# Intelligent-Microsystems-Lab/SNNQuantPrune

Measured on AMD Instinct MI355X. Metric: samples/sec/node (DVS128 T=20, 4-bit/90%-pruned), higher is better.
Workload: dtype fp6*fp4->f32 (integer-exact); 1 GPU; C3 topology: 3x(qconv3x3+BN+LIF+pool2) + qdense(32768->110)+LIF + vote, DVS128 128x128x2, T=20, bits 4/4/4/4, 90% pruned; batch_per_gpu=1024, global_batch=1024, frames=20, parallelism=dp1 (batch-sharded, all-gather logits)

## Files before the change

include/snnqp.h:

```cpp
#ifndef SNNQP_H_
#define SNNQP_H_

#include <stdint.h>

#ifdef __cplusplus
extern "C" {
#endif

typedef void *snnqp_stream_t;

enum {
  SNNQP_OK = 0,
  SNNQP_EINVAL = -1,
  SNNQP_EUNSUPPORTED = -2,
  SNNQP_EHIP = -3
};

enum { SNNQP_F32 = 0, SNNQP_U8 = 1, SNNQP_BITS = 2, SNNQP_EV1 = 3, SNNQP_EV4 = 4 };
enum { SNNQP_W_F32 = 0, SNNQP_W_I8 = 1 };
enum {
  SNNQP_NEURON_NONE = 0,
  SNNQP_NEURON_MULTI_STEP_LIF = 1,
  SNNQP_NEURON_PARAMETRIC_LEAKY_IF = 2,
  SNNQP_NEURON_LIF = 3
};
enum {
  SNNQP_SURR_FAST_SIGMOID = 0,
  SNNQP_SURR_ATAN = 1,
  SNNQP_SURR_SLAYER = 2,
  SNNQP_SURR_SMOOTH_STEP = 3,
  SNNQP_SURR_PIECEWISE_LINEAR = 4
};
enum {
  SNNQP_Q_DUQ = 0,
  SNNQP_Q_UNIFORM_STATIC = 1,
  SNNQP_Q_PARAMETRIC_D = 2,
  SNNQP_Q_PARAMETRIC_D_XMAX = 3
};
enum { SNNQP_IMPL_AUTO = 0, SNNQP_IMPL_GENERIC = 1, SNNQP_IMPL_MFMA = 2 };

enum {
  SNNQP_FLAG_CODE_OVERFLOW = 1,
  SNNQP_FLAG_MASK_NOT_BINARY = 2,
  SNNQP_FLAG_NOT_INTEGER = 4,
  SNNQP_FLAG_GT_ONE = 8,
  SNNQP_FLAG_GT_127 = 16,
  SNNQP_FLAG_GT_15 = 32
};

typedef struct {
  int32_t wtype;
  const void *w;
  float L;
  float m;
  int32_t abs_sum_max;
  int32_t code_max;
  const int32_t *col_sum;
  const void *wt_fp6;
  uint32_t min_current_bits;
  int32_t ch_stack_max;
  const int32_t *ch_slots;
  int32_t wt_cin;
} snnqp_weight_t;

#define SNNQP_BN_MEAN_ZERO 1
#define SNNQP_BN_BIAS_ZERO 2
#define SNNQP_BN_MUL_UNIFORM 4
typedef struct {
  const float *mean;
  const float *mul;
  const float *bias;
  int32_t flags;
} snnqp_bn_t;

typedef struct {
  int32_t kind;
  float k;
  float v_threshold;
  float v_reset;
  const float *decay;
} snnqp_neuron_t;

typedef struct {
  int32_t H, W, Cin, Cout;
  int32_t KH, KW;
  int32_t stride_h, stride_w;
  int32_t pad_h_lo, pad_h_hi, pad_w_lo, pad_w_hi;
  int32_t in_dil_h, in_dil_w;
  int32_t k_dil_h, k_dil_w;
  int32_t groups;
} snnqp_conv_geom_t;

typedef struct {
  int32_t D, H, W, Cin, Cout;
  int32_t KD, KH, KW;
  int32_t stride[3];
  int32_t pad_lo[3], pad_hi[3];
  int32_t in_dil[3];
  int32_t k_dil[3];
  int32_t groups;
} snnqp_conv3d_geom_t;

#define SNNQP_VERSION 507
int snnqp_version(void);
const char *snnqp_last_error(void);
const char *snnqp_build_flags(void);

int snnqp_set_conv_k16(int enabled);

int snnqp_conv_out_shape(const snnqp_conv_geom_t *g, int32_t *OH, int32_t *OW);

int snnqp_quantize(int kind, const float *w, const float *mask, int64_t n,
                   int bits, float p0, float p1, float *fq_out,
                   int8_t *codes_out, int32_t *flags, snnqp_stream_t stream);
int snnqp_quantize_ex(int kind, const float *w, const float *mask, int64_t n,
                      int bits, int sign, float p0, float p1, float *fq_out,
                      int8_t *codes_out, int32_t *flags, snnqp_stream_t stream);

int snnqp_pack_codes_mfma(const int8_t *w, int64_t K, int32_t N, int32_t Npad,
                          int8_t *wt, snnqp_stream_t stream);

int snnqp_pack_codes_fp6(const int8_t *w, int64_t K, int32_t N, int32_t Npad, void *wt6,
                         snnqp_stream_t stream);

int snnqp_inspect_f32(const float *x, int64_t n, int32_t *flags,
                      snnqp_stream_t stream);
int snnqp_inspect_u8(const uint8_t *x, int64_t n, int32_t *flags,
                     snnqp_stream_t stream);
int snnqp_f32_to_u8(const float *x, uint8_t *y, int64_t n,
                    snnqp_stream_t stream);
int snnqp_narrow_f32(const float *x, uint8_t *y, int64_t n, int32_t *flags,
                     snnqp_stream_t stream);
int snnqp_pack_frames(const uint8_t *x, int64_t frames, int32_t H, int32_t W, int fmt,
                      void *y, int32_t *flags, snnqp_stream_t stream);
int snnqp_unpack_frames(const void *x, int fmt, int64_t frames, int32_t H, int32_t W,
                        uint8_t *y, snnqp_stream_t stream);
int snnqp_pack_frames_checked(const void *x, int in_type, int64_t frames, int32_t H, int32_t W,
                              uint32_t *y, int32_t *flags, snnqp_stream_t stream);
int snnqp_pack_bits(const void *x, int in_type, int64_t rows, int32_t C,
                    uint32_t *bits, snnqp_stream_t stream);
int snnqp_pack_bits_checked(const void *x, int in_type, int64_t rows, int32_t C,
                            uint32_t *bits, int32_t *flags, snnqp_stream_t stream);
int snnqp_unpack_bits(const uint32_t *bits, int64_t rows, int32_t C, float *y,
                      snnqp_stream_t stream);

int snnqp_conv_forward(const void *x, int in_type, int64_t NB,
                       const snnqp_conv_geom_t *g, const snnqp_weight_t *w,
                       float *y, int32_t *acc, snnqp_stream_t stream);
int snnqp_conv_forward_ex(const void *x, int in_type, int64_t NB,
                          const snnqp_conv_geom_t *g, const snnqp_weight_t *w,
                          const int8_t *wt, float *y, int32_t *acc, int impl,
                          snnqp_stream_t stream);
int snnqp_conv_forward_if(const int32_t *pred, const void *x, int in_type, int64_t NB,
                          const snnqp_conv_geom_t *g, const snnqp_weight_t *w, float *y,
                          snnqp_stream_t stream);

int snnqp_conv3d_out_shape(const snnqp_conv3d_geom_t *g, int32_t *OD, int32_t *OH, int32_t *OW);
int snnqp_conv3d_lif_forward(const int32_t *pred, const void *x, int in_type, int64_t x_stride_t,
                             int64_t x_stride_b, int32_t T, int32_t B,
                             const snnqp_conv3d_geom_t *g, const snnqp_weight_t *w,
                             const snnqp_bn_t *bn, const snnqp_neuron_t *nrn, const float *u0,
                             float *u_out, void *s_out, int s_type, snnqp_stream_t stream);

int64_t snnqp_conv_gated_packed_bytes(int32_t Cin, int32_t Cout);
int snnqp_pack_codes_gated(const int8_t *w, int32_t Cin, int32_t Cout, void *packed,
                           snnqp_stream_t stream);
int64_t snnqp_conv_gated_packed_bytes_ex(int32_t Cin, int32_t Cout, int32_t code_max);
int snnqp_pack_codes_gated_ex(const int8_t *w, int32_t Cin, int32_t Cout, int32_t code_max,
                              void *packed, snnqp_stream_t stream);
int snnqp_conv_gated_forward(const uint32_t *s, const float *gate, int64_t NB,
                             const snnqp_conv_geom_t *g, const snnqp_weight_t *w,
                             const void *packed, float *y, snnqp_stream_t stream);

int64_t snnqp_dense_gated_packed_bytes(int32_t C, int32_t N);
int snnqp_pack_codes_dense_gated(const int8_t *w, int32_t C, int32_t HW, int32_t N, void *packed,
                                 snnqp_stream_t stream);
int64_t snnqp_dense_gated_packed_bytes_ex(int32_t C, int32_t N, int32_t code_max);
int snnqp_pack_codes_dense_gated_ex(const int8_t *w, int32_t C, int32_t HW, int32_t N, int32_t code_max,
                                    void *packed, snnqp_stream_t stream);
int snnqp_dense_gated_forward(const uint32_t *s, const float *gate, int64_t NB, int32_t HW,
                              int32_t C, int32_t N, const snnqp_weight_t *w,
                              const void *packed, float *y, snnqp_stream_t stream);

int snnqp_conv_lif_forward(const void *x, int in_type, int64_t x_stride_t,
                           int64_t x_stride_b, int32_t T, int32_t B,
                           const snnqp_conv_geom_t *g, const snnqp_weight_t *w,
                           const int8_t *wt, const snnqp_bn_t *bn,
                           const snnqp_neuron_t *nrn, const float *u0,
                           float *u_out, void *s_out, int s_type, int pool,
                           int impl, int x_max, int32_t *x_seen, int32_t *x_flags,
                           snnqp_stream_t stream);
// ... 130 lines not shown
```

snnquantprune_amd/_lib.py:

```python

from __future__ import annotations

import ctypes
import os
from ctypes import (POINTER, Structure, c_char_p, c_float, c_int, c_int8,
                    c_int32, c_uint32, c_int64, c_void_p)

_HERE = os.path.dirname(os.path.abspath(__file__))
LIB_PATH = os.path.join(_HERE, "csrc", "libsnnqp.so")

ABI_VERSION = 507

F32, U8, BITS, EV1, EV4 = 0, 1, 2, 3, 4
W_F32, W_I8 = 0, 1
NEURON_NONE, NEURON_MULTI_STEP_LIF, NEURON_PARAMETRIC_LEAKY_IF, NEURON_LIF = 0, 1, 2, 3
SURR_FAST_SIGMOID, SURR_ATAN, SURR_SLAYER, SURR_SMOOTH_STEP, SURR_PIECEWISE_LINEAR = 0, 1, 2, 3, 4
Q_DUQ, Q_UNIFORM_STATIC, Q_PARAMETRIC_D, Q_PARAMETRIC_D_XMAX = 0, 1, 2, 3
IMPL_AUTO, IMPL_GENERIC, IMPL_MFMA = 0, 1, 2
FLAG_CODE_OVERFLOW, FLAG_MASK_NOT_BINARY = 1, 2
FLAG_NOT_INTEGER, FLAG_GT_ONE, FLAG_GT_127, FLAG_GT_15 = 4, 8, 16, 32
OK, EINVAL, EUNSUPPORTED, EHIP = 0, -1, -2, -3
STATUS_QUEUE_CORRUPT, STATUS_TICKET, STATUS_BOUND = 1, 2, 4


class WeightT(Structure):
  _fields_ = [("wtype", c_int32), ("w", c_void_p), ("L", c_float), ("m", c_float),
              ("abs_sum_max", c_int32), ("code_max", c_int32), ("col_sum", c_void_p),
              ("wt_fp6", c_void_p), ("min_current_bits", c_uint32), ("ch_stack_max", c_int32),
              ("ch_slots", c_void_p), ("wt_cin", c_int32)]


BN_MEAN_ZERO, BN_BIAS_ZERO, BN_MUL_UNIFORM = 1, 2, 4


class BnT(Structure):
  _fields_ = [("mean", c_void_p), ("mul", c_void_p), ("bias", c_void_p), ("flags", c_int32)]


class NeuronT(Structure):
  _fields_ = [("kind", c_int32), ("k", c_float), ("v_threshold", c_float),
              ("v_reset", c_float), ("decay", c_void_p)]


class ConvGeomT(Structure):
  _fields_ = [(n, c_int32) for n in (
      "H", "W", "Cin", "Cout", "KH", "KW", "stride_h", "stride_w",
      "pad_h_lo", "pad_h_hi", "pad_w_lo", "pad_w_hi",
      "in_dil_h", "in_dil_w", "k_dil_h", "k_dil_w", "groups")]


class Conv3dGeomT(Structure):
  _fields_ = ([(n, c_int32) for n in ("D", "H", "W", "Cin", "Cout", "KD", "KH", "KW")]
              + [(n, c_int32 * 3) for n in ("stride", "pad_lo", "pad_hi", "in_dil", "k_dil")]
              + [("groups", c_int32)])


_PROTOTYPES = {
    "snnqp_version": (c_int, []),
    "snnqp_last_error": (c_char_p, []),
    "snnqp_build_flags": (c_char_p, []),
    "snnqp_set_conv_k16": (c_int, [c_int]),
    "snnqp_conv_out_shape": (c_int, [POINTER(ConvGeomT), POINTER(c_int32),
                                     POINTER(c_int32)]),
    "snnqp_quantize": (c_int, [c_int, c_void_p, c_void_p, c_int64, c_int, c_float,
                               c_float, c_void_p, c_void_p, c_void_p, c_void_p]),
    "snnqp_quantize_ex": (c_int, [c_int, c_void_p, c_void_p, c_int64, c_int, c_int, c_float,
                                  c_float, c_void_p, c_void_p, c_void_p, c_void_p]),
    "snnqp_pack_codes_mfma": (c_int, [c_void_p, c_int64, c_int32, c_int32, c_void_p,
                                      c_void_p]),
    "snnqp_pack_codes_fp6": (c_int, [c_void_p, c_int64, c_int32, c_int32, c_void_p, c_void_p]),
    "snnqp_inspect_f32": (c_int, [c_void_p, c_int64, c_void_p, c_void_p]),
    "snnqp_inspect_u8": (c_int, [c_void_p, c_int64, c_void_p, c_void_p]),
    "snnqp_f32_to_u8": (c_int, [c_void_p, c_void_p, c_int64, c_void_p]),
    "snnqp_narrow_f32": (c_int, [c_void_p, c_void_p, c_int64, c_void_p, c_void_p]),
    "snnqp_pack_frames": (c_int, [c_void_p, c_int64, c_int32, c_int32, c_int, c_void_p, c_void_p,
                                  c_void_p]),
    "snnqp_unpack_frames": (c_int, [c_void_p, c_int, c_int64, c_int32, c_int32, c_void_p,
                                    c_void_p]),
    "snnqp_pack_bits": (c_int, [c_void_p, c_int, c_int64, c_int32, c_void_p,
                                c_void_p]),
    "snnqp_pack_bits_checked": (c_int, [c_void_p, c_int, c_int64, c_int32, c_void_p, c_void_p,
                                        c_void_p]),
    "snnqp_unpack_bits": (c_int, [c_void_p, c_int64, c_int32, c_void_p, c_void_p]),
    "snnqp_conv_forward": (c_int, [c_void_p, c_int, c_int64, POINTER(ConvGeomT),
                                   POINTER(WeightT), c_void_p, c_void_p, c_void_p]),
    "snnqp_conv_forward_ex": (c_int, [c_void_p, c_int, c_int64, POINTER(ConvGeomT),
                                      POINTER(WeightT), c_void_p, c_void_p, c_void_p, c_int, c_void_p]),
    "snnqp_conv_forward_if": (c_int, [c_void_p, c_void_p, c_int, c_int64, POINTER(ConvGeomT),
                                      POINTER(WeightT), c_void_p, c_void_p]),
    "snnqp_conv3d_out_shape": (c_int, [POINTER(Conv3dGeomT), POINTER(c_int32), POINTER(c_int32),
                                       POINTER(c_int32)]),
    "snnqp_conv3d_lif_forward": (c_int, [
        c_void_p, c_void_p, c_int, c_int64, c_int64, c_int32, c_int32, POINTER(Conv3dGeomT),
        POINTER(WeightT), POINTER(BnT), POINTER(NeuronT), c_void_p, c_void_p, c_void_p, c_int, c_void_p]),
    "snnqp_conv_gated_packed_bytes": (c_int64, [c_int32, c_int32]),
    "snnqp_pack_codes_gated": (c_int, [c_void_p, c_int32, c_int32, c_void_p, c_void_p]),
    "snnqp_conv_gated_packed_bytes_ex": (c_int64, [c_int32, c_int32, c_int32]),
    "snnqp_pack_codes_gated_ex": (c_int, [c_void_p, c_int32, c_int32, c_int32, c_void_p, c_void_p]),
    "snnqp_conv_gated_forward": (c_int, [c_void_p, c_void_p, c_int64, POINTER(ConvGeomT),
                                         POINTER(WeightT), c_void_p, c_void_p, c_void_p]),
    "snnqp_dense_gated_packed_bytes": (c_int64, [c_int32, c_int32]),
    "snnqp_pack_codes_dense_gated": (c_int, [c_void_p, c_int32, c_int32, c_int32, c_void_p, c_void_p]),
    "snnqp_dense_gated_packed_bytes_ex": (c_int64, [c_int32, c_int32, c_int32]),
    "snnqp_pack_codes_dense_gated_ex": (c_int, [c_void_p, c_int32, c_int32, c_int32, c_int32, c_void_p, c_void_p]),
    "snnqp_dense_gated_forward": (c_int, [c_void_p, c_void_p, c_int64, c_int32, c_int32, c_int32,
                                          POINTER(WeightT), c_void_p, c_void_p, c_void_p]),
    "snnqp_conv_lif_forward": (c_int, [
        c_void_p, c_int, c_int64, c_int64, c_int32, c_int32, POINTER(ConvGeomT),
        POINTER(WeightT), c_void_p, POINTER(BnT), POINTER(NeuronT), c_void_p,
        c_void_p, c_void_p, c_int, c_int, c_int, c_int, c_void_p, c_void_p, c_void_p]),
    "snnqp_conv_lif_forward_pred": (c_int, [
        c_void_p, c_void_p, c_int, c_int64, c_int64, c_int32, c_int32, POINTER(ConvGeomT),
        POINTER(WeightT), c_void_p, POINTER(BnT), POINTER(NeuronT), c_void_p,
        c_void_p, c_void_p, c_int, c_int, c_int, c_void_p, c_void_p, c_void_p]),
    "snnqp_pack_frames_checked": (c_int, [c_void_p, c_int, c_int64, c_int32, c_int32, c_void_p, c_void_p,
                                          c_void_p]),
    "snnqp_conv_lif_forward_if": (c_int, [
        c_void_p, c_void_p, c_int, c_int64, c_int64, c_int32, c_int32, POINTER(ConvGeomT),
        POINTER(WeightT), POINTER(BnT), POINTER(NeuronT), c_void_p, c_void_p, c_void_p, c_int, c_int,
        c_void_p]),
    "snnqp_dense_lif_forward_if": (c_int, [
        c_void_p, c_void_p, c_int, c_int64, c_int64, c_int32, c_int32, c_int32, c_int32,
        POINTER(WeightT), POINTER(BnT), POINTER(NeuronT), c_void_p, c_void_p, c_void_p, c_int,
        c_void_p]),
    "snnqp_dense_lif_forward": (c_int, [
        c_void_p, c_int, c_int64, c_int64, c_int32, c_int32, c_int32, c_int32,
        POINTER(WeightT), c_void_p, POINTER(BnT), POINTER(NeuronT), c_void_p,
        c_void_p, c_void_p, c_int, c_int, c_void_p]),
    "snnqp_dense_workspace_bytes": (c_int64, [c_int, c_int32, c_int32, c_int32, c_int32, POINTER(WeightT)]),
    "snnqp_dense_lif_forward_ws": (c_int, [
        c_void_p, c_int, c_int64, c_int64, c_int32, c_int32, c_int32, c_int32,
        POINTER(WeightT), c_void_p, POINTER(BnT), POINTER(NeuronT), c_void_p,
        c_void_p, c_void_p, c_int, c_int, c_void_p, c_void_p, c_int64, c_void_p]),
    "snnqp_dense_head_workspace_bytes": (c_int64, [c_int32, c_int32, c_int32]),
    "snnqp_dense_head_forward": (c_int, [
        c_void_p, c_int, c_int64, c_int64, c_int32, c_int32, c_int32, c_int32, POINTER(WeightT),
        c_void_p, POINTER(NeuronT), c_int32, POINTER(WeightT), c_void_p, POINTER(NeuronT), c_int32,
        c_void_p, c_void_p, c_void_p, c_void_p, c_void_p, c_int64, c_void_p]),
    "snnqp_device_status": (c_int, [c_int, POINTER(c_uint32), c_int]),
    "snnqp_workqueue_capture_mark": (c_int, [c_int, POINTER(c_int64)]),
    "snnqp_workqueue_capture_release": (c_int, [c_int, c_int64, c_int64]),
    "snnqp_workqueue_stats": (c_int, [POINTER(c_int64), POINTER(c_int64), POINTER(c_int64), c_int]),
    "snnqp_debug_workqueue_poke": (c_int, [c_int, c_int64, c_int, c_uint32]),
    "snnqp_fallback_counts": (c_int, [POINTER(c_int64), POINTER(c_int64), c_char_p, c_int32, c_int]),
# ... 93 lines not shown
```

snnquantprune_amd/csrc/api.hip:

```cpp
#include <atomic>

#include "common.h"

namespace snnqp {

static std::atomic<int> g_conv_k16{1};
bool conv_k16_enabled() { return g_conv_k16.load(std::memory_order_relaxed) != 0; }

static thread_local std::string g_last_error;

void set_error(const char *fmt, ...) {
  char buf[512];
  va_list ap;
  va_start(ap, fmt);
  vsnprintf(buf, sizeof(buf), fmt, ap);
  va_end(ap);
  g_last_error = buf;
}

}

extern "C" {

int snnqp_version(void) { return SNNQP_VERSION; }

const char *snnqp_last_error(void) { return snnqp::g_last_error.c_str(); }

#ifndef SNNQP_BUILD_FLAGS
#define SNNQP_BUILD_FLAGS ""
#endif
const char *snnqp_build_flags(void) { return SNNQP_BUILD_FLAGS; }

int snnqp_set_conv_k16(int enabled) {
  if (enabled < 0) return snnqp::conv_k16_enabled() ? 1 : 0;
  return snnqp::g_conv_k16.exchange(enabled ? 1 : 0, std::memory_order_relaxed);
}

int snnqp_conv_out_shape(const snnqp_conv_geom_t *g, int32_t *OH, int32_t *OW) {
  SNNQP_REQUIRE(g && OH && OW, SNNQP_EINVAL, "conv_out_shape: null argument");
  SNNQP_REQUIRE(g->stride_h > 0 && g->stride_w > 0 && g->in_dil_h > 0 &&
                    g->in_dil_w > 0 && g->k_dil_h > 0 && g->k_dil_w > 0 &&
                    g->KH > 0 && g->KW > 0,
                SNNQP_EINVAL, "conv_out_shape: non-positive stride/dilation/kernel");
  const int64_t hd = g->H > 0 ? (int64_t)(g->H - 1) * g->in_dil_h + 1 : 0;
  const int64_t wd = g->W > 0 ? (int64_t)(g->W - 1) * g->in_dil_w + 1 : 0;
  const int64_t kh = (int64_t)(g->KH - 1) * g->k_dil_h + 1;
  const int64_t kw = (int64_t)(g->KW - 1) * g->k_dil_w + 1;
  const int64_t th = hd + g->pad_h_lo + g->pad_h_hi;
  const int64_t tw = wd + g->pad_w_lo + g->pad_w_hi;
  *OH = th < kh ? 0 : (int32_t)((th - kh) / g->stride_h + 1);
  *OW = tw < kw ? 0 : (int32_t)((tw - kw) / g->stride_w + 1);
  return SNNQP_OK;
}

}
```

snnquantprune_amd/csrc/blocks.hip:

```cpp
#include "common.h"
#include "kernels.h"

#include <atomic>
#include <cstdlib>
#include <cstring>
#include <mutex>

using namespace snnqp;

namespace {
std::atomic<int64_t> g_fallback_conv{0}, g_fallback_dense{0};
std::mutex g_fallback_mu;
char g_fallback_reason[256] = "";

void note_fallback(bool dense, const char *why) {
  (dense ? g_fallback_dense : g_fallback_conv).fetch_add(1, std::memory_order_relaxed);
  static const bool log = std::getenv("SNNQP_LOG_FALLBACKS") != nullptr;
  std::lock_guard<std::mutex> lock(g_fallback_mu);
  const bool fresh = std::strncmp(g_fallback_reason + (dense ? 7 : 6), why ? why : "", 200) != 0;
  std::snprintf(g_fallback_reason, sizeof(g_fallback_reason), "%s%s", dense ? "dense: " : "conv: ",
                why ? why : "");
  if (log && fresh)
    std::fprintf(stderr, "libsnnqp: %s block on the direct-form kernel: %s\n",
                 dense ? "dense" : "conv", why ? why : "");
}

snnqp_conv_geom_t dense_geom(int32_t K, int32_t N) {
  snnqp_conv_geom_t g;
  g.H = 1; g.W = 1; g.Cin = K; g.Cout = N; g.KH = 1; g.KW = 1;
  g.stride_h = g.stride_w = 1;
  g.pad_h_lo = g.pad_h_hi = g.pad_w_lo = g.pad_w_hi = 0;
  g.in_dil_h = g.in_dil_w = g.k_dil_h = g.k_dil_w = 1;
  g.groups = 1;
  return g;
}

#define SNNQP_CHECK_NEURON_KIND(nrn, who)                                                      \
  SNNQP_REQUIRE((nrn)->kind >= SNNQP_NEURON_MULTI_STEP_LIF && (nrn)->kind <= SNNQP_NEURON_LIF, \
                SNNQP_EINVAL, who ": unknown neuron kind %d", (nrn)->kind)
}

extern "C" {

int snnqp_fallback_counts(int64_t *conv_blocks, int64_t *dense_blocks, char *reason,
                          int32_t reason_len, int reset) {
  if (conv_blocks) *conv_blocks = g_fallback_conv.load(std::memory_order_relaxed);
  if (dense_blocks) *dense_blocks = g_fallback_dense.load(std::memory_order_relaxed);
  std::lock_guard<std::mutex> lock(g_fallback_mu);
  if (reason && reason_len > 0) {
    std::strncpy(reason, g_fallback_reason, (size_t)reason_len - 1);
    reason[reason_len - 1] = 0;
  }
  if (reset) {
    g_fallback_conv = 0;
    g_fallback_dense = 0;
    g_fallback_reason[0] = 0;
  }
  return SNNQP_OK;
}

int snnqp_conv_dequant_form(const snnqp_weight_t *w, const snnqp_neuron_t *nrn) {
  SNNQP_REQUIRE(w && nrn, SNNQP_EINVAL, "conv_dequant_form: null descriptor");
  SNNQP_REQUIRE(w->wtype == SNNQP_W_I8, SNNQP_EINVAL, "conv_dequant_form: int8 codes only");
  return conv3x3_bits_dequant_form(w, nrn);
}

int snnqp_conv_lif_forward(const void *x, int in_type, int64_t x_stride_t,
                           int64_t x_stride_b, int32_t T, int32_t B,
                           const snnqp_conv_geom_t *g, const snnqp_weight_t *w,
                           const int8_t *wt, const snnqp_bn_t *bn,
                           const snnqp_neuron_t *nrn,
                           const float *u0, float *u_out, void *s_out,
                           int s_type, int pool, int impl, int x_max, int32_t *x_seen,
                           int32_t *x_flags, snnqp_stream_t stream) {
  SNNQP_REQUIRE(g && w && nrn, SNNQP_EINVAL, "conv_lif_forward: null descriptor");
  if (in_type == SNNQP_F32 && w->wtype == SNNQP_W_I8)
    SNNQP_REQUIRE(x_flags != nullptr, SNNQP_EINVAL,
                  "conv_lif_forward: float32 input into integer codes needs x_flags (snnqp.h)");
  if (int rc = refuse_after_device_report((hipStream_t)stream, "conv_lif_forward")) return rc;
  SNNQP_CHECK_NEURON_KIND(nrn, "conv_lif_forward");
  SNNQP_REQUIRE(pool == 1 || pool == 2, SNNQP_EINVAL,
                "conv_lif_forward: pool must be 1 or 2");
  SNNQP_REQUIRE(impl >= SNNQP_IMPL_AUTO && impl <= SNNQP_IMPL_MFMA, SNNQP_EINVAL,
                "conv_lif_forward: unknown impl %d", impl);
  const char *why = conv3x3_mfma_unsupported(in_type, g, w, wt, nrn, s_type);
  if (impl == SNNQP_IMPL_MFMA)
    SNNQP_REQUIRE(!why, SNNQP_EUNSUPPORTED, "conv_lif_forward: MFMA kernel: %s", why);
  if (!why && impl != SNNQP_IMPL_GENERIC)
    return run_conv3x3_mfma(x, in_type, x_stride_t, x_stride_b, T, B, g, w, wt, bn,
                            nrn, u0, u_out, (uint32_t *)s_out, pool, x_max, x_seen, x_flags,
                            (hipStream_t)stream);
  SNNQP_REQUIRE(in_type != SNNQP_EV1 && in_type != SNNQP_EV4, SNNQP_EUNSUPPORTED,
                "conv_lif_forward: packed event frames need bit-packed spike output; unpack them first "
                "(%s)", why ? why : "impl = GENERIC");
  SNNQP_REQUIRE(!(in_type == SNNQP_F32 && w->wtype == SNNQP_W_I8), SNNQP_EUNSUPPORTED,
                "conv_lif_forward: float32 input into integer codes is staged by the event-layer MFMA "
                "kernel only (%s); narrow it first (snnqp_narrow_f32 / snnqp_pack_bits_checked)",
                why ? why : "impl = GENERIC");
  SNNQP_REQUIRE(pool == 1, SNNQP_EUNSUPPORTED,
                "conv_lif_forward: the direct-form kernel does not fuse the "
                "max-pool; call snnqp_maxpool2x2 after it");
  if (impl == SNNQP_IMPL_AUTO) note_fallback(false, why);
  return run_generic(x, in_type, x_stride_t, x_stride_b, T, B, g, w, bn, nrn, u0,
                     u_out, s_out, s_type, nullptr, (hipStream_t)stream);
}

int snnqp_conv_lif_forward_pred(const int32_t *pred, const void *x, int in_type, int64_t x_stride_t,
                                int64_t x_stride_b, int32_t T, int32_t B,
                                const snnqp_conv_geom_t *g, const snnqp_weight_t *w,
                                const int8_t *wt, const snnqp_bn_t *bn,
                                const snnqp_neuron_t *nrn,
                                const float *u0, float *u_out, void *s_out,
                                int s_type, int pool, int x_max, int32_t *x_seen,
                                int32_t *x_flags, snnqp_stream_t stream) {
  SNNQP_REQUIRE(pred && g && w && nrn, SNNQP_EINVAL, "conv_lif_forward_pred: null argument");
  if (in_type == SNNQP_F32 && w->wtype == SNNQP_W_I8)
    SNNQP_REQUIRE(x_flags != nullptr, SNNQP_EINVAL,
                  "conv_lif_forward_pred: float32 input into integer codes needs x_flags (snnqp.h)");
  if (int rc = refuse_after_device_report((hipStream_t)stream, "conv_lif_forward_pred")) return rc;
  SNNQP_CHECK_NEURON_KIND(nrn, "conv_lif_forward_pred");
  SNNQP_REQUIRE(pool == 1 || pool == 2, SNNQP_EINVAL, "conv_lif_forward_pred: pool must be 1 or 2");
  SNNQP_REQUIRE(in_type == SNNQP_U8 || in_type == SNNQP_F32 || in_type == SNNQP_EV4, SNNQP_EUNSUPPORTED,
                "conv_lif_forward_pred: byte, nibble or float32 frames (the event layer's own formats)");
  const char *why = conv3x3_mfma_unsupported(in_type, g, w, wt, nrn, s_type);
  SNNQP_REQUIRE(!why, SNNQP_EUNSUPPORTED, "conv_lif_forward_pred: MFMA kernel: %s", why);
  return run_conv3x3_mfma(x, in_type, x_stride_t, x_stride_b, T, B, g, w, wt, bn, nrn, u0, u_out,
                          (uint32_t *)s_out, pool, x_max, x_seen, x_flags, (hipStream_t)stream, pred);
}

int snnqp_conv_lif_forward_if(const int32_t *pred, const void *x, int in_type, int64_t x_stride_t,
                              int64_t x_stride_b, int32_t T, int32_t B,
                              const snnqp_conv_geom_t *g, const snnqp_weight_t *w,
                              const snnqp_bn_t *bn, const snnqp_neuron_t *nrn, const float *u0,
                              float *u_out, void *s_out, int s_type, int pool,
                              snnqp_stream_t stream) {
  SNNQP_REQUIRE(pred && g && w && nrn, SNNQP_EINVAL, "conv_lif_forward_if: null argument");
  if (int rc = refuse_after_device_report((hipStream_t)stream, "conv_lif_forward_if")) return rc;
  SNNQP_CHECK_NEURON_KIND(nrn, "conv_lif_forward_if");
  SNNQP_REQUIRE(pool == 1 || pool == 2, SNNQP_EINVAL, "conv_lif_forward_if: pool must be 1 or 2");
  return run_generic(x, in_type, x_stride_t, x_stride_b, T, B, g, w, bn, nrn, u0, u_out, s_out, s_type,
                     nullptr, (hipStream_t)stream, pool, pred);
}

int snnqp_dense_lif_forward_if(const int32_t *pred, const void *x, int in_type, int64_t x_stride_t,
                               int64_t x_stride_b, int32_t T, int32_t B, int32_t K, int32_t N,
                               const snnqp_weight_t *w, const snnqp_bn_t *bn,
                               const snnqp_neuron_t *nrn, const float *u0, float *u_out,
// ... 87 lines not shown
```

snnquantprune_amd/csrc/conv3x3_u8c2.hip:

```cpp
#include <atomic>
#include <map>
#include <mutex>
#include <tuple>
#include <type_traits>
#include <utility>

#include <vector>

#include "conv_tile.h"

namespace snnqp {

constexpr int HROW2 = 24;
constexpr int HCOPY2 = HALO * HROW2;
constexpr int HCONST2 = 2 * HCOPY2;
constexpr int HIMG2 = 496;
constexpr int TCHUNK = 32;
constexpr int U8C2_WPS = 4;
constexpr int STG_N = TCHUNK / 2;

typedef int v2i_a4 __attribute__((ext_vector_type(2), aligned(4)));
typedef __attribute__((address_space(3))) const v2i_a4 lds_cv2i_t;

__host__ __device__ inline int u8c2_table_bytes(int lutm, int bound, int rows) {
  const int b = lutm == LUT_CHANNEL ? rows * 128 : lutm == LUT_SHARED ? (2 * bound + 2) * 4 : 0;
  return (b + 15) & ~15;
}

#ifndef SNNQP_U8C2_EV1_WPS
#define SNNQP_U8C2_EV1_WPS 5
#endif
#ifndef SNNQP_U8C2_ONE_WPS
#define SNNQP_U8C2_ONE_WPS 4
#endif
#ifndef SNNQP_U8C2_EV1_ONE_WPS
#define SNNQP_U8C2_EV1_ONE_WPS 6
#endif
template <int NF, bool POOL, int LUTM, int IN, bool ONE>
constexpr int u8c2_waves() {
  if (IN == SNNQP_EV1 && ONE && LUTM == LUT_CHANNEL && NF == NF_MUL0 && POOL) return SNNQP_U8C2_EV1_ONE_WPS;
  if (IN == SNNQP_EV1) return SNNQP_U8C2_EV1_WPS;
  return ONE ? SNNQP_U8C2_ONE_WPS : U8C2_WPS;
}
template <int NF, bool POOL, int LUTM, int IN = SNNQP_U8, bool ONE = false>
__global__ void __launch_bounds__(256, (u8c2_waves<NF, POOL, LUTM, IN, ONE>()))
conv3x3_u8c2_kernel(ConvMfmaArgs a) {
  constexpr int FL = OutStage<POOL>::FL;
  constexpr bool EV1 = IN == SNNQP_EV1;
  constexpr bool EV4 = IN == SNNQP_EV4;
  constexpr bool F32IN = IN == SNNQP_F32;
  static_assert(TCHUNK % FL == 0, "flush period must divide the staging chunk");
  if constexpr (!EV1) {
    if (a.pred && *(const volatile int32_t *)a.pred == 0) return;
  }
  extern __shared__ __attribute__((aligned(16))) uint8_t lds[];
  const int tc = a.tchunk;
  const int lut_off = tc * HIMG2;
  uint32_t *obuf = (uint32_t *)(lds + lut_off + u8c2_table_bytes(LUTM, a.lut_bound, a.lut_rows));
  const int tid = threadIdx.x, lane = tid & 63;
  const int wave = __builtin_amdgcn_readfirstlane(tid >> 6);
  const int n = lane & 31, h = lane >> 5;
  const int cout_base = blockIdx.y * 128 + wave * 32;
  const bool wave_on = cout_base < a.Cout;
  const int cout = wave_on ? cout_base + n : n;
  const int cpar = cout < a.Cout ? cout : a.Cout - 1;
  const uint32_t cmask = chan_mask(cout_base, a.Cout);
  uint32_t *wgw = obuf + OutStage<POOL>::BYTES / 4;
  if (tid == 0) { wgw[0] = 0x7F800000u; wgw[1] = 0u; }
  typedef int v2i_a8 __attribute__((ext_vector_type(2)));
  v2i_a8 *xtab = (v2i_a8 *)(wgw + 4);
  if (EV1) {
    const uint32_t one = LUTM == LUT_CHANNEL ? 16u : LUTM == LUT_SHARED ? 4u : 0x81u;
    const uint32_t zero = LUTM == LUT_NONE ? 0x80u : 0u;
    uint32_t e[2] = {0, 0};
#pragma unroll
    for (int j = 0; j < 8; ++j) e[j >> 2] |= (((uint32_t)tid >> j) & 1u ? one : zero) << (8 * (j & 3));
    xtab[tid] = v2i_a8{(int)e[0], (int)e[1]};
  }
  if (LUTM != LUT_NONE) lds_barrier();
  if (LUTM == LUT_SHARED) {
    build_lut((float *)(lds + lut_off), a.lut_bound, a.dq, tid);
    if (NF == NF_MUL0) {
      lds_barrier();
      atomicMin(wgw, lut_bn_min_bits((const float *)(lds + lut_off), a.lut_bound, a.bn,
                                     blockIdx.y * 128, a.Cout, tid, 256));
    }
  }
  int ch_row0 = 0, ch_col = 0;
  if (LUTM == LUT_CHANNEL) {
    int pos = 0, neg = 0;
#pragma unroll
    for (int j = 0; j < 16; ++j) {
      const int k = 16 * h + j, dy = k >> 3, b = k & 7;
      if (k < 24 && b < 6 && wave_on && cout < a.Cout) {
        const int code = a.w[(int64_t)(6 * dy + b) * a.Cout + cout];
        pos += code > 0 ? code : 0;
        neg += code < 0 ? -code : 0;
      }
    }
    pos += __shfl_xor(pos, 32);
    neg += __shfl_xor(neg, 32);
    uint32_t *scr = obuf;
    int slot = 4 * n + wave;
    if (a.ch_slots) slot = a.ch_slots[blockIdx.y * 128 + wave * 32 + n] & 127;
    if (h == 0) {
      scr[slot] = (uint32_t)((pos + neg) * a.x_limit + 1);
      scr[128 + wave * 32 + n] = (uint32_t)(neg * a.x_limit);
      scr[256 + wave * 32 + n] = (uint32_t)slot;
    }
    lds_barrier();
    ch_col = slot >> 2;
    const int start = lut_column_start(scr, slot);
    int total = 0;
#pragma unroll
    for (int k = 0; k < 4; ++k) total += (int)scr[(slot & ~3) + k];
    ch_row0 = start + neg * a.x_limit;
    if (total > a.lut_rows && a.status) *(volatile uint32_t *)a.status = SNNQP_STATUS_BOUND;
    const uint32_t mb = build_lut_channel((float *)(lds + lut_off), scr, a.lut_rows, a.dq, a.bn,
                                          blockIdx.y * 128, a.Cout, tid);
    atomicMin(wgw, mb);
    lds_barrier();
  }
  if (tid < tc) {
    *(uint32_t *)(lds + tid * HIMG2 + HCONST2) = 0x7F7F7F7Fu;
    *(uint32_t *)(lds + tid * HIMG2 + HCONST2 + 4) = 0x00000001u;
  }

  float acc_off = 0.0f;
  v4i bf, bfg;
  {
    int bias = 0;
    if (LUTM == LUT_SHARED) bias = (int)lds_addr(lds) + lut_off + 4 * a.lut_bound;
    if (LUTM == LUT_CHANNEL)
      bias = (int)lds_addr(lds) + lut_off + 4 * (ch_row0 * 32 + ch_col);
    int q = bias / 127;
    const int r = bias - 127 * q;
    int wsum = 0;
    int v[4], vg[4];
#pragma unroll
    for (int d = 0; d < 4; ++d) {
      uint32_t pk = 0, pkg = 0;
#pragma unroll
      for (int j = 0; j < 4; ++j) {
        const int k = 16 * h + 4 * d + j;
        uint32_t bv = 0, bg = 0;
        if (k < 24) {
          const int dy = k >> 3, b = k & 7;
          if (b < 6 && cout < a.Cout) {
            const int code = a.w[(int64_t)(6 * dy + b) * a.Cout + cout];
            wsum += code;
            bg = (uint8_t)code;
            bv = (uint8_t)(LUTM == LUT_CHANNEL ? code * 8 : code);
          }
        } else if (k < 28) {
          const int part = q < 127 ? q : 127;
          q -= part;
          bv = (uint32_t)part;
        } else if (k == 28) {
          bv = (uint32_t)r;
        }
        pk |= bv << (8 * j);
        pkg |= bg << (8 * j);
      }
      v[d] = (int)pk;
      vg[d] = (int)pkg;
    }
    bf = v4i{v[0], v[1], v[2], v[3]};
    bfg = v4i{vg[0], vg[1], vg[2], vg[3]};
    acc_off = 128.0f * (float)(wsum + __shfl_xor(wsum, 32));
  }

  LaneConsts lc = {0.f, 1.f, 0.f, 0.f, a.nrn.vr};
  if (a.bn.mean) { lc.bmean = a.bn.mean[cpar]; lc.bmul = a.bn.mul[cpar]; lc.bbias = a.bn.bias[cpar]; }
  if (a.nrn.kind == SNNQP_NEURON_LIF) lc.dec = a.nrn.decay[cpar];

  const int ty = ((n >> 2) & 1) | ((n >> 4) << 1);
  const int tx = (n & 3) | (((n >> 3) & 1) << 2);
  const int cpy = tx & 1;
  const int px0 = (int)lds_addr(lds) + cpy * HCOPY2 + 2 * tx + 2 * cpy;
  int offA[2], offB[2];
#pragma unroll
  for (int tl = 0; tl < 2; ++tl) {
    offA[tl] = px0 + (ty + 4 * tl + (h ? 2 : 0)) * HROW2;
    offB[tl] = h ? (int)lds_addr(lds) + HCONST2 : px0 + (ty + 4 * tl + 1) * HROW2;
  }
  const uint8_t *xb = (const uint8_t *)a.x;
  const int ob0 = out_pix<POOL>(0, lane) * 4 + wave;
  const int ob1 = out_pix<POOL>(1, lane) * 4 + wave;
  const bool store_lane = POOL ? lane < 8 : lane < 32;
  uint32_t seen = 0;
  uint32_t hist[6] = {0, 0, 0, 0, 0, 0};
  const int s_pix = tid & 127;
  const bool s_task = s_pix < HALO * HALO;
  const int s_half = __builtin_amdgcn_readfirstlane(tid >> 7);
  const int s_dst = (s_pix / HALO) * HROW2 + (s_pix % HALO) * 2;

  PatchWalk pw(a);
  int r = __builtin_amdgcn_readfirstlane((int)pw.first);
  uint32_t processed = 0;
  while (r < (int)pw.count) {
    ++processed;
    int claimed = 0;
    if (pw.queue && tid == 0) claimed = (int)pw.claim();
    int b, y0, x0;
    pw.decode(a, r, b, y0, x0);

    float u[2][16];
    if constexpr (!ONE) {
      if (a.u0 && wave_on) u_io<true>(u, a, b, y0, x0, cout, h);
      else zero_u(u);
    }
    uint32_t pseen = 0;
    const int s_gy = y0 + s_pix / HALO - 1, s_gx = x0 + s_pix % HALO - 1;
    const bool s_valid = s_task && s_gy >= 0 && s_gy < a.H && s_gx >= 0 && s_gx < a.W;
    const uint32_t s_off = s_valid ? (uint32_t)(s_gy * a.W + s_gx) * (EV4 ? 1u : F32IN ? 8u : 2u) : 0u;
    const uint8_t *s_frames = xb + (int64_t)b * a.xs_b * (F32IN ? 4 : 1);
    const uint32_t e_lead = x0 > 0 ? 2u : 0u;
    const int e_hi = min(HALO - 1, a.W - x0);
    const uint32_t e_colmask = ((1u << (2 * (e_hi + 1))) - 1u) & ~((1u << (2 - (int)e_lead)) - 1u);
    const uint32_t e_fwords = (uint32_t)(((int64_t)a.H * a.W * 2 + 31) >> 5);
    const uint32_t *e_frames = (const uint32_t *)a.x + (int64_t)b * a.xs_b;

    for (int t0 = 0; t0 < a.T; t0 += tc) {
      const int nt = min(tc, a.T - t0);
      bool general = LUTM == LUT_NONE;
      if constexpr (EV1) {
        lds_barrier();
        for (int task = tid; task < nt * HALO; task += 256) {
          const int tt = task / HALO, hy = task - tt * HALO;
          const int gy = y0 + hy - 1;
          const bool rv = gy >= 0 && gy < a.H;
          const uint32_t start = (uint32_t)((rv ? gy : 0) * a.W + x0) * 2u - e_lead;
          const uint32_t wi = start >> 5;
          const uint32_t *f = e_frames + (int64_t)(t0 + tt) * a.xs_t;
          const uint32_t lo = f[wi], hi = f[min(wi + 1u, e_fwords - 1u)];
          uint32_t v = __builtin_amdgcn_alignbit(hi, lo, start & 31u);
          v = (v << (2u - e_lead)) & (rv ? e_colmask : 0u);
          const v2i_a8 d0 = xtab[v & 0xFFu], d1 = xtab[(v >> 8) & 0xFFu], d2 = xtab[(v >> 16) & 0xFu];
          uint8_t *row = lds + tt * HIMG2 + hy * HROW2;
          *(v2i_a8 *)row = d0;
          *(v2i_a8 *)(row + 8) = d1;
          *(v2i_a8 *)(row + 16) = d2;
          const uint32_t q0 = (uint32_t)d0.x, q1 = (uint32_t)d0.y, q2 = (uint32_t)d1.x,
                         q3 = (uint32_t)d1.y, q4 = (uint32_t)d2.x, q5 = (uint32_t)d2.y;
          uint8_t *row1 = row + HCOPY2;
          *(v2i_a8 *)row1 = v2i_a8{(int)(q0 << 16), (int)__builtin_amdgcn_alignbit(q1, q0, 16)};
          *(v2i_a8 *)(row1 + 8) = v2i_a8{(int)__builtin_amdgcn_alignbit(q2, q1, 16),
                                         (int)__builtin_amdgcn_alignbit(q3, q2, 16)};
          *(v2i_a8 *)(row1 + 16) = v2i_a8{(int)__builtin_amdgcn_alignbit(q4, q3, 16),
                                          (int)__builtin_amdgcn_alignbit(q5, q4, 16)};
        }
        lds_barrier();
      } else {
      uint32_t v[STG_N];
      uint32_t mx = 0;
      if constexpr (F32IN) {
        uint32_t fbad = 0;
#pragma unroll
        for (int r0 = 0; r0 < STG_N; r0 += STG_N / 2) {
          typedef float f2v __attribute__((ext_vector_type(2)));
          f2v raw[STG_N / 2];
#pragma unroll
          for (int i = r0; i < r0 + STG_N / 2; ++i) {
            const int tt = 2 * i + s_half;
            raw[i - r0] = f2v{0.0f, 0.0f};
            if (tt < nt) raw[i - r0] = *(const f2v *)(s_frames + (int64_t)(t0 + tt) * a.xs_t * 4 + s_off);
          }
#pragma unroll
          for (int i = r0; i < r0 + STG_N / 2; ++i) {
            const f2v f = raw[i - r0];
            const uint32_t ua = __float2uint_rz(f.x), ub = __float2uint_rz(f.y);
            fbad |= __float_as_uint(__uint2float_rn(ua) - f.x) | __float_as_uint(__uint2float_rn(ub) - f.y);
// ... 4 lines not shown
        fbad = s_valid ? fbad : 0u;
        if (__ballot(fbad != 0u) != 0ull && lane == 0 && a.x_flags) atomicOr(a.x_flags, SNNQP_FLAG_NOT_INTEGER);
      } else {
#pragma unroll
      for (int i = 0; i < STG_N; ++i) {
        const int tt = 2 * i + s_half;
        v[i] = 0;
        if (tt < nt) {
          if constexpr (EV4) {
            const uint32_t pb = *(s_frames + (int64_t)(t0 + tt) * a.xs_t + s_off);
            v[i] = (pb | (pb << 4)) & 0x0F0Fu;
          } else {
            v[i] = *(const uint16_t *)(s_frames + (int64_t)(t0 + tt) * a.xs_t + s_off);
          }
        }
      }
      }
#pragma unroll
      for (int i = 0; i < STG_N; ++i) {
        v[i] = s_valid ? v[i] : 0u;
        mx = max(mx, max(v[i] & 0xFFu, v[i] >> 8));
      }
#pragma unroll
      for (int off = 32; off > 0; off >>= 1) mx = max(mx, (uint32_t)__shfl_xor((int)mx, off));
      if (tid == 0) wgw[1] = 0u;
      lds_barrier();
      if (s_task) {
#pragma unroll
        for (int i = 0; i < STG_N; ++i) {
          const int tt = 2 * i + s_half;
          if (tt < nt) {
            const uint16_t val = (uint16_t)(LUTM == LUT_NONE      ? v[i] ^ 0x8080u
                                            : LUTM == LUT_CHANNEL ? v[i] << 4
                                                                  : v[i] << 2);
            uint8_t *p = lds + tt * HIMG2 + s_dst;
            *(uint16_t *)p = val;
            *(uint16_t *)(p + HCOPY2 + 2) = val;
          }
        }
      }
      if (lane == 0 && mx != 0) atomicMax(&wgw[1], mx);
      lds_barrier();
      const uint32_t cmax = (uint32_t)__builtin_amdgcn_readfirstlane((int)wgw[1]);
      seen = max(seen, cmax);
      pseen = max(pseen, cmax);
      hist[0] += cmax <= 1u;
      hist[1] += cmax == 2u;
      hist[2] += cmax > 2u && cmax <= 7u;
      hist[3] += cmax > 7u && cmax <= 31u;
      hist[4] += cmax > 31u;
      hist[5] += cmax == 3u;
      general = LUTM == LUT_NONE || cmax > (uint32_t)a.x_limit;
      if (LUTM != LUT_NONE && general) {
        if (s_task) {
#pragma unroll 1
          for (int tt = s_half; tt < nt; tt += 2) {
            uint32_t w2 = 0;
            if (s_valid) {
              if constexpr (F32IN) {
                typedef float f2v __attribute__((ext_vector_type(2)));
                const f2v f = *(const f2v *)(s_frames + (int64_t)(t0 + tt) * a.xs_t * 4 + s_off);
                w2 = (__float2uint_rz(f.x) & 0xFFu) | ((__float2uint_rz(f.y) & 0xFFu) << 8);
              } else if constexpr (EV4) {
                const uint32_t pb = *(s_frames + (int64_t)(t0 + tt) * a.xs_t + s_off);
                w2 = (pb | (pb << 4)) & 0x0F0Fu;
              } else {
                w2 = *(const uint16_t *)(s_frames + (int64_t)(t0 + tt) * a.xs_t + s_off);
              }
            }
            const uint16_t val = (uint16_t)(w2 ^ 0x8080u);
            uint8_t *p = lds + tt * HIMG2 + s_dst;
            *(uint16_t *)p = val;
            *(uint16_t *)(p + HCOPY2 + 2) = val;
          }
        }
        lds_barrier();
      }
      }
      auto run_chunk = [&](auto mode_tag, auto fma_tag) {
      constexpr int MODE = decltype(mode_tag)::value;
      constexpr bool FMA = decltype(fma_tag)::value;
      constexpr bool OFFS = MODE == LUT_NONE;
      const v4i bw = OFFS ? bfg : bf;
      for (int tf = 0; tf < nt; tf += FL) {
        const int nf = min(FL, nt - tf);
#pragma unroll 1
        for (int tt = tf; tt < (wave_on ? tf + nf : tf); ++tt) {
          const uint32_t img = (uint32_t)(tt * HIMG2);
          uint32_t words[2];
#pragma unroll
          for (int tl = 0; tl < 2; ++tl) {
            const v2i_a4 lo = *(lds_cv2i_t *)(uintptr_t)(img + (uint32_t)offA[0] + (uint32_t)(tl * 4 * HROW2));
            const v2i_a4 hi = *(lds_cv2i_t *)(uintptr_t)(img + (uint32_t)offB[tl]);
            v16i acc = splat16(0);
            acc = __builtin_amdgcn_mfma_i32_32x32x32_i8(v4i{lo.x, lo.y, hi.x, hi.y}, bw, acc,
                                                        0, 0, 0);
            if constexpr (u8c2_waves<NF, POOL, LUTM, IN, ONE>() >= 6)
              words[tl] = tile_epilogue_halves<NF, POOL, MODE, FMA, OFFS>(acc, u[tl], a.dq, lc, a.nrn,
                                                                            lane, acc_off);
            else
              words[tl] = tile_epilogue<NF, POOL, MODE, FMA, OFFS>(acc, u[tl], a.dq, lc, a.nrn,
                                                                     lane, acc_off);
          }
          if (store_lane) {
            uint32_t *o = obuf + ((t0 + tt) % FL) * (OutStage<POOL>::NPIX * 4);
            o[ob0] = words[0] & cmask;
            o[ob0 + (POOL ? 32 : 128)] = words[1] & cmask;
          }
        }
        lds_barrier();
        flush_out<POOL>(obuf, a, t0 + tf, nf, b, y0, x0, tid);
        lds_barrier();
      }
      };
      if constexpr (ONE) zero_u(u);
      if (general) {
        run_chunk(std::integral_constant<int, LUT_NONE>{}, std::false_type{});
      } else if constexpr (LUTM != LUT_NONE) {
        const bool fma_ok = NF == NF_MUL0 && pseen <= (uint32_t)a.x_limit &&
                            lif_fma_is_exact(wgw[0], a.nrn.k_log2, a.T, a.u0 != nullptr);
        if (fma_ok) run_chunk(std::integral_constant<int, LUTM>{}, std::true_type{});
        else run_chunk(std::integral_constant<int, LUTM>{}, std::false_type{});
      }
      if constexpr (ONE) break;
    }
    if (!ONE && a.u_out && wave_on) u_io<false>(u, a, b, y0, x0, cout, h);
    int r_next = r + (int)pw.stride;
    if (pw.queue) {
      if (tid == 0) wgw[2] = (uint32_t)claimed;
      lds_barrier();
      r_next = __builtin_amdgcn_readfirstlane((int)wgw[2]);
    }
    r = r_next;
  }
  if (a.x_seen && tid == 0) {
    if (seen != 0) atomicMax(a.x_seen, seen);
#pragma unroll
    for (int k = 0; k < 6; ++k)
      if (hist[k] != 0) atomicAdd((uint32_t *)a.x_seen + 1 + k, hist[k]);
  }
  if (pw.queue && tid == 0) pw.finish(processed, a.npatch, a.status);
}


__global__ void __launch_bounds__(256)
current_min_kernel(Dequant dq, BnP bn, int bound, int Cout, uint32_t *out) {
  const int c = blockIdx.x * 64 + (threadIdx.x & 63);
  uint32_t mb = 0x7F800000u;
  if (c < Cout) {
    float mean = 0.f, mul = 1.f, bias = 0.f;
    if (bn.mean) { mean = bn.mean[c]; mul = bn.mul[c]; bias = bn.bias[c]; }
    for (int i = (int)(threadIdx.x >> 6) + 4 * (int)blockIdx.y - bound; i <= bound; i += 4 * (int)gridDim.y) {
      float x = dequant_acc(i, dq) - mean;
      x = x * mul;
      x = x + bias;
      const uint32_t b = __float_as_uint(x) & 0x7FFFFFFFu;
      if (b != 0 && b < mb) mb = b;
    }
  }
  for (int off = 32; off > 0; off >>= 1) {
    const uint32_t o = (uint32_t)__shfl_xor((int)mb, off);
    mb = o < mb ? o : mb;
  }
  if ((threadIdx.x & 63) == 0 && mb != 0x7F800000u) atomicMin(out, mb);
}

// ... 120 lines not shown
void persistent_limits(const void *kernel, int threads, size_t dyn_lds, int dev, int *cus_out,
                       int *occ_out) {
  typedef std::tuple<const void *, int, size_t, int> Key;
  static std::mutex mu;
  static std::map<Key, std::pair<int, int>> cache;
  const Key key(kernel, threads, dyn_lds, dev);
  std::lock_guard<std::mutex> lock(mu);
  auto it = cache.find(key);
  if (it == cache.end()) {
    int cus = 256, occ = 1;
    DeviceGuard on(dev);
    if (hipDeviceGetAttribute(&cus, hipDeviceAttributeMultiprocessorCount, dev) != hipSuccess) {
      (void)hipGetLastError();
      cus = 256;
    }
    if (hipOccupancyMaxActiveBlocksPerMultiprocessor(&occ, kernel, threads, dyn_lds) != hipSuccess) {
      (void)hipGetLastError();
      occ = 1;
    }
    if (occ < 1) occ = 1;
    if (occ > 8) occ = 8;
    it = cache.emplace(key, std::make_pair(cus, occ)).first;
  }
  *cus_out = it->second.first;
  *occ_out = it->second.second;
}

int run_current_min(const snnqp_weight_t *w, const snnqp_bn_t *bn, int32_t bound, int32_t Cout,
                    uint32_t *out_bits, hipStream_t st) {
  SNNQP_REQUIRE(w && out_bits && Cout > 0 && bound >= 0, SNNQP_EINVAL, "current_min: bad argument");
  SNNQP_REQUIRE(w->L >= 1.0f, SNNQP_EINVAL, "dequant L must be >= 1");
  SNNQP_CHECK_BN(bn);
  const int slices = bound >= 256 ? 16 : 1;
  hipLaunchKernelGGL(current_min_kernel, dim3((Cout + 63) / 64, slices), dim3(256), 0, st,
                     make_dequant(w->L, w->m), make_bn(bn), bound, Cout, out_bits);
  SNNQP_CHECK_LAUNCH("current_min_kernel");
  return SNNQP_OK;
}

const char *conv3x3_mfma_unsupported(int in_type, const snnqp_conv_geom_t *g,
                                     const snnqp_weight_t *w, const int8_t *wt,
                                     const snnqp_neuron_t *nrn, int s_type) {
  if (w->wtype != SNNQP_W_I8) return "weights are not int8 codes";
  if (g->KH != 3 || g->KW != 3) return "kernel is not 3x3";
  if (g->stride_h != 1 || g->stride_w != 1) return "stride is not 1";
  if (g->pad_h_lo != 1 || g->pad_h_hi != 1 || g->pad_w_lo != 1 || g->pad_w_hi != 1)
    return "padding is not ((1,1),(1,1))";
  if (g->in_dil_h != 1 || g->in_dil_w != 1 || g->k_dil_h != 1 || g->k_dil_w != 1)
    return "dilated convolution";
  if (g->groups != 1) return "grouped convolution";
  if (g->H <= 0 || g->W <= 0) return "empty image";
  if (g->Cout <= 0) return "no output channels";
  if (s_type != SNNQP_BITS) return "spike output must be bit-packed";
  if (in_type == SNNQP_BITS) {
    if (g->Cin < 1 || g->Cin > 128) return "bit input needs Cin <= 128";
  } else if (in_type == SNNQP_U8) {
    if (g->Cin != 2) return "u8 input needs Cin == 2";
    if ((int64_t)g->H * g->W * 2 >= (int64_t)1 << 31) return "u8 frame of 2 GiB or more";
  } else if (in_type == SNNQP_EV1) {
    if (g->Cin != 2) return "EV1 frames have Cin == 2";
    if ((int64_t)g->H * g->W * 2 >= (int64_t)1 << 31) return "EV1 frame of 2^31 bits or more";
  } else if (in_type == SNNQP_EV4) {
    if (g->Cin != 2) return "EV4 frames have Cin == 2";
    if ((int64_t)g->H * g->W >= (int64_t)1 << 31) return "EV4 frame of 2 GiB or more";
  } else if (in_type == SNNQP_F32) {
    if (g->Cin != 2) return "float32 input into integer codes needs Cin == 2";
    if ((int64_t)g->H * g->W * 8 >= (int64_t)1 << 31) return "float32 frame of 2 GiB or more";
  } else {
    return "input must be BITS, U8, EV1, EV4 or (Cin == 2) F32";
  }
  if (nrn->kind == SNNQP_NEURON_LIF && !nrn->decay) return "LIF without decay";
  if (in_type == SNNQP_BITS && !wt) return "MFMA-tiled codes `wt` not given";
  return nullptr;
}

int conv3x3_bits_dequant_form(const snnqp_weight_t *w, const snnqp_neuron_t *nrn) {
  if (w->L == 1.0f) return DQ_ONE;
  const bool fp6 = w->code_max > 0 && w->code_max <= 7;
  const bool tab = fp6 && neuron_form(make_neuron(nrn)) == NF_MUL0 && w->abs_sum_max > 0 &&
                   w->abs_sum_max <= DQT_MAXA;
  return tab ? DQ_TABLE : DQ_ARITH;
}

int run_conv3x3_mfma(const void *x, int in_type, int64_t xs_t, int64_t xs_b,
                     int32_t T, int32_t B, const snnqp_conv_geom_t *g,
                     const snnqp_weight_t *w, const int8_t *wt,
                     const snnqp_bn_t *bn, const snnqp_neuron_t *nrn,
                     const float *u0, float *u_out, uint32_t *s_out, int pool,
                     int x_max, int32_t *x_seen, int32_t *x_flags, hipStream_t st, const int32_t *pred) {
  SNNQP_REQUIRE(w->w && ((x && s_out) || T == 0 || B == 0), SNNQP_EINVAL, "conv3x3 mfma: null pointer");
  SNNQP_REQUIRE(!pred || in_type == SNNQP_U8 || in_type == SNNQP_F32 || in_type == SNNQP_EV4, SNNQP_EUNSUPPORTED,
                "conv3x3 mfma: only the event layer on byte / nibble / float32 frames takes a predicate");
  SNNQP_REQUIRE(in_type != SNNQP_BITS || wt, SNNQP_EINVAL,
                "conv3x3 mfma: bit input needs the MFMA-tiled codes `wt`");
  const int cin_pad = w->wt_cin ? w->wt_cin : (g->Cin + 31) / 32 * 32;
  SNNQP_REQUIRE(in_type != SNNQP_BITS || (cin_pad % 32 == 0 && cin_pad >= g->Cin && cin_pad <= 128),
                SNNQP_EINVAL, "conv3x3 mfma: wt_cin must be a multiple of 32 in [Cin, 128]");
  SNNQP_REQUIRE(T >= 0 && B >= 0, SNNQP_EINVAL, "conv3x3 mfma: negative T/B");
  SNNQP_REQUIRE(w->L >= 1.0f, SNNQP_EINVAL, "dequant L must be >= 1");
  SNNQP_CHECK_BN(bn);
  if (T == 0 || B == 0) return SNNQP_OK;
  SNNQP_REQUIRE((int64_t)B * ((g->H + 3) / 4) * ((g->W + 7) / 8) < ((int64_t)1 << 30),
                SNNQP_EUNSUPPORTED, "conv3x3 mfma: more than 2^30 patches in one launch");
  ConvMfmaArgs a;
  a.x = x; a.xs_t = xs_t; a.xs_b = xs_b; a.T = T; a.B = B;
  a.H = g->H; a.W = g->W; a.Cin = g->Cin; a.Cout = g->Cout;
  a.w = (const int8_t *)w->w;
  a.wt = wt;
  a.dq = make_dequant(w->L, w->m);
  a.bn = make_bn(bn);
  a.nrn = make_neuron(nrn);
  a.u0 = u0; a.u_out = u_out; a.s_out = s_out; a.pool = pool;
  a.x_seen = x_seen;
  a.x_flags = nullptr;
  a.pred = pred;
  if (in_type == SNNQP_F32) {
    SNNQP_REQUIRE(x_flags != nullptr && (((uintptr_t)x) & 7) == 0 && xs_t % 2 == 0 && xs_b % 2 == 0,
                  SNNQP_EINVAL, "conv3x3 mfma: float32 frames need x_flags and 8-byte aligned pixels");
    if (int rc = zero_words_async((uint32_t *)x_flags, 1, st)) return rc;
    a.x_flags = x_flags;
  }
  a.patch_h = 8;
  a.tiles_y = (g->H + 7) / 8; a.tiles_x = (g->W + 7) / 8;
  a.npatch = (int64_t)B * a.tiles_y * a.tiles_x;
  const int nf = neuron_form(a.nrn);
  const bool pl = pool == 2;
  const unsigned gy = (unsigned)((g->Cout + 127) / 128);
  const bool ev1 = in_type == SNNQP_EV1;
  const int64_t xm = (in_type == SNNQP_BITS || ev1) ? 1 : (x_max > 0 ? x_max : 1);
  a.x_limit = (int32_t)(xm > 255 ? 255 : xm);
  const int64_t bound = (int64_t)w->abs_sum_max * xm;
  const bool lut = w->abs_sum_max > 0 && xm > 0 && xm <= LUT_XMAX && bound <= LUT_CAP;
  a.lut_bound = lut ? (int32_t)bound : 0;
  a.tchunk = T >= TCHUNK ? TCHUNK : T;
  const size_t lds_fixed = (size_t)a.tchunk * HIMG2 + 16 + (ev1 ? 2048 : 0) +
                           (pl ? OutStage<true>::BYTES : OutStage<false>::BYTES);
  const int64_t stack = w->ch_stack_max > 0 ? (int64_t)w->ch_stack_max : 8 * (int64_t)w->abs_sum_max;
  const int64_t crows = stack * xm + 4;
  const bool lutc = lut && in_type != SNNQP_BITS && crows <= LUT2_ROWS && xm <= 7 &&
                    w->code_max > 0 && w->code_max <= 15;
  a.lut_rows = lutc ? (int32_t)crows : 0;
  a.ch_slots = lutc && w->ch_stack_max > 0 ? w->ch_slots : nullptr;
#define SNNQP_CONV_LAUNCH_IN(KERN, NFV, PL, LM, LDS)                               \
  do {                                                                             \
    if (ev1 && one) launch_persistent(KERN<NFV, PL, LM, SNNQP_EV1, true>, a, gy, st, LDS); \
    else if (ev1) launch_persistent(KERN<NFV, PL, LM, SNNQP_EV1>, a, gy, st, LDS);       \
    else if (in_type == SNNQP_EV4 && one) launch_persistent(KERN<NFV, PL, LM, SNNQP_EV4, true>, a, gy, st, LDS); \
    else if (in_type == SNNQP_EV4) launch_persistent(KERN<NFV, PL, LM, SNNQP_EV4>, a, gy, st, LDS); \
    else if (in_type == SNNQP_F32 && one) launch_persistent(KERN<NFV, PL, LM, SNNQP_F32, true>, a, gy, st, LDS); \
    else if (in_type == SNNQP_F32) launch_persistent(KERN<NFV, PL, LM, SNNQP_F32>, a, gy, st, LDS); \
    else if (one) launch_persistent(KERN<NFV, PL, LM, SNNQP_U8, true>, a, gy, st, LDS);            \
    else launch_persistent(KERN<NFV, PL, LM, SNNQP_U8>, a, gy, st, LDS);            \
  } while (0)
#define SNNQP_CONV_LAUNCH_NF(KERN, NFV, LM, LDS)                                   \
  do {                                                                             \
    if (pl) SNNQP_CONV_LAUNCH_IN(KERN, NFV, true, LM, LDS);                         \
    else SNNQP_CONV_LAUNCH_IN(KERN, NFV, false, LM, LDS);                           \
  } while (0)
#define SNNQP_CONV_LAUNCH(KERN, LM, LDS)                                           \
  do {                                                                             \
    if (nf == NF_MUL0) SNNQP_CONV_LAUNCH_NF(KERN, NF_MUL0, LM, LDS);                \
    else if (nf == NF_MUL) SNNQP_CONV_LAUNCH_NF(KERN, NF_MUL, LM, LDS);             \
    else if (nf == NF_DIV) SNNQP_CONV_LAUNCH_NF(KERN, NF_DIV, LM, LDS);             \
    else SNNQP_CONV_LAUNCH_NF(KERN, NF_DECAY, LM, LDS);                             \
  } while (0)
  if (in_type == SNNQP_BITS) {
    const bool fma = nf == NF_MUL0 && w->min_current_bits != 0 && w->abs_sum_max > 0 &&
                     lif_fma_is_exact(w->min_current_bits, a.nrn.k_log2, T, u0 != nullptr);
    const bool i8 = !(w->code_max > 0 && w->code_max <= 7);
    int dq = conv3x3_bits_dequant_form(w, nrn);
    if (dq == DQ_TABLE && !dq_table_trusted(stream_device(st), st)) dq = DQ_ARITH;
    const bool tab = dq == DQ_TABLE;
    const bool bnf = (a.bn.flags & (SNNQP_BN_MEAN_ZERO | SNNQP_BN_BIAS_ZERO)) ==
                     (SNNQP_BN_MEAN_ZERO | SNNQP_BN_BIAS_ZERO);
    a.lut_bound = tab ? (int32_t)w->abs_sum_max : 0;
    if (tab) check_code_bound_once(stream_device(st), (const int8_t *)w->w, (int64_t)9 * g->Cin, g->Cout,
                                   w->abs_sum_max, st);
    const int cin16 = (g->Cin + 15) / 16 * 16;
    const int cin_walk = conv_k16_enabled() && cin16 + 16 == cin_pad ? cin16 : cin_pad;
    launch_conv3x3_bits(a, cin_walk, i8, nf, pl, dq, fma, bnf, gy, st);
  } else {
    const int lm = lutc ? LUT_CHANNEL : lut ? LUT_SHARED : LUT_NONE;
    if (lut) check_code_bound_once(stream_device(st), (const int8_t *)w->w, (int64_t)9 * g->Cin, g->Cout,
                                   w->abs_sum_max, st);
    const size_t lds_rest = lds_fixed - (size_t)a.tchunk * HIMG2 + u8c2_table_bytes(lm, a.lut_bound, a.lut_rows);
    for (int wgs = 4; wgs >= 2; --wgs) {
      const size_t per_wg = (size_t)(160 * 1024) / wgs - 512;
      int tc = a.tchunk;
      while (tc > 16 && (size_t)tc * HIMG2 + lds_rest > per_wg) tc -= 1;
      if ((size_t)tc * HIMG2 + lds_rest <= per_wg) {
        a.tchunk = tc;
        break;
      }
    }
    const size_t ldsb = (size_t)a.tchunk * HIMG2 + lds_rest;
    const bool one = !a.u0 && !a.u_out && a.T <= a.tchunk;
    if (lutc) SNNQP_CONV_LAUNCH(conv3x3_u8c2_kernel, LUT_CHANNEL, ldsb);
    else if (lut) SNNQP_CONV_LAUNCH(conv3x3_u8c2_kernel, LUT_SHARED, ldsb);
    else SNNQP_CONV_LAUNCH(conv3x3_u8c2_kernel, LUT_NONE, ldsb);
  }
#undef SNNQP_CONV_LAUNCH
#undef SNNQP_CONV_LAUNCH_NF
#undef SNNQP_CONV_LAUNCH_IN
  SNNQP_CHECK_LAUNCH("conv3x3 mfma kernel");
  return SNNQP_OK;
}

}

extern "C" int snnqp_workqueue_capture_mark(int device, int64_t *mark) {
  using namespace snnqp;
  SNNQP_REQUIRE(device >= 0 && device < 64 && mark, SNNQP_EINVAL, "workqueue_capture_mark: bad argument");
  std::lock_guard<std::mutex> lock(g_sched_mu);
  *mark = (int64_t)g_sched[device].capture_log.size();
  return SNNQP_OK;
}

extern "C" int snnqp_workqueue_capture_release(int device, int64_t mark_begin, int64_t mark_end) {
  using namespace snnqp;
  SNNQP_REQUIRE(device >= 0 && device < 64, SNNQP_EINVAL, "workqueue_capture_release: bad device");
  std::lock_guard<std::mutex> lock(g_sched_mu);
  SchedPool &p = g_sched[device];
  SNNQP_REQUIRE(0 <= mark_begin && mark_begin <= mark_end && mark_end <= (int64_t)p.capture_log.size(),
                SNNQP_EINVAL, "workqueue_capture_release: marks out of range");
  for (int64_t i = mark_begin; i < mark_end; ++i) {
    const int slot = p.capture_log[(size_t)i];
    if (slot < 0) continue;
    p.capture_free.push_back(slot);
    p.capture_log[(size_t)i] = -1;
  }
  return SNNQP_OK;
}

extern "C" int snnqp_workqueue_stats(int64_t *captured_static, int64_t *busy_static,
                                     int64_t *dequant_fallbacks, int reset) {
  using namespace snnqp;
  if (captured_static) *captured_static = g_static_captured.load(std::memory_order_relaxed);
  if (busy_static) *busy_static = g_static_busy.load(std::memory_order_relaxed);
  if (dequant_fallbacks) *dequant_fallbacks = dq_table_fallbacks(reset != 0);
  if (reset) { g_static_captured = 0; g_static_busy = 0; }
  return SNNQP_OK;
}

extern "C" int snnqp_debug_workqueue_poke(int device, int64_t mark, int word, uint32_t value) {
  using namespace snnqp;
  SNNQP_REQUIRE(device >= 0 && device < 64 && word >= 0 && word < SCHED_WORDS, SNNQP_EINVAL,
                "debug_workqueue_poke: bad argument");
  std::lock_guard<std::mutex> lock(g_sched_mu);
  SchedPool &p = g_sched[device];
  SNNQP_REQUIRE(p.words && mark >= 0 && mark < (int64_t)p.capture_log.size() && p.capture_log[(size_t)mark] >= 0,
                SNNQP_EINVAL, "debug_workqueue_poke: no live capture slot at mark %lld", (long long)mark);
  SNNQP_HIP(hipMemcpy(p.words + (size_t)p.capture_log[(size_t)mark] * SCHED_WORDS + word, &value, 4,
                      hipMemcpyHostToDevice));
  return SNNQP_OK;
}
```

snnquantprune_amd/csrc/conv_tile.h:

```cpp
#pragma once
#include "kernels.h"

namespace snnqp {

struct v2f {
  float x, y;
};
__device__ __forceinline__ v2f operator+(v2f a, v2f b) { return v2f{a.x + b.x, a.y + b.y}; }
__device__ __forceinline__ v2f operator-(v2f a, v2f b) { return v2f{a.x - b.x, a.y - b.y}; }
__device__ __forceinline__ v2f operator*(v2f a, v2f b) { return v2f{a.x * b.x, a.y * b.y}; }
__device__ __forceinline__ v2f operator+(v2f a, float b) { return v2f{a.x + b, a.y + b}; }
__device__ __forceinline__ v2f operator-(v2f a, float b) { return v2f{a.x - b, a.y - b}; }
__device__ __forceinline__ v2f operator*(v2f a, float b) { return v2f{a.x * b, a.y * b}; }
__device__ __forceinline__ v2f operator-(v2f a) { return v2f{-a.x, -a.y}; }
__device__ __forceinline__ v2f fma2(v2f a, v2f b, v2f c) {
  return v2f{__builtin_fmaf(a.x, b.x, c.x), __builtin_fmaf(a.y, b.y, c.y)};
}


enum { LUT_NONE = 0, LUT_SHARED = 1, LUT_CHANNEL = 2 };
constexpr int LUT_CAP = 4095;
constexpr int LUT2_ROWS = 256;
constexpr int LUT_XMAX = 31;

constexpr int HALO = 10;
constexpr int HPITCH = 12;
constexpr int HPLANE = HALO * HPITCH * 32;

typedef __attribute__((address_space(3))) const v4i lds_cv4i_t;

constexpr int F6_PITCH = HPITCH;
constexpr int F6_ROWS = 6;
constexpr int F6_NT = 256;
constexpr int F6_PLANE = F6_ROWS * HPITCH * 32;
constexpr int F6_TAB = FP4_TAB_BYTES;

__device__ __forceinline__ void fp6_pack32(const v4i &lo, const v4i &hi, int (&d)[6]) {
  uint32_t t[8];
#pragma unroll
  for (int i = 0; i < 4; ++i) {
    t[i] = squeeze6(fp6_codes4((uint32_t)lo[i]));
    t[4 + i] = squeeze6(fp6_codes4((uint32_t)hi[i]));
  }
#pragma unroll
  for (int g = 0; g < 2; ++g) {
    d[3 * g + 0] = (int)(t[4 * g] | (t[4 * g + 1] << 24));
    d[3 * g + 1] = (int)((t[4 * g + 1] >> 8) | (t[4 * g + 2] << 16));
    d[3 * g + 2] = (int)((t[4 * g + 2] >> 16) | (t[4 * g + 3] << 8));
  }
}

enum { FMT_FP6 = 0, FMT_I8 = 1 };

__host__ __device__ constexpr int pair_tap(int p, int h) { return p < 3 ? p + 3 * h : 2 * p + h; }

struct ConvMfmaArgs {
  const void *x;
  int64_t xs_t, xs_b;
  int32_t T, B, H, W, Cin, Cout;
  const int8_t *w;
  const int8_t *wt;
  Dequant dq;
  BnP bn;
  NeuronP nrn;
  const float *u0;
  float *u_out;
  uint32_t *s_out;
  int32_t pool;
  int32_t tiles_y, tiles_x;
  int64_t npatch;
  int32_t lut_bound;
  int32_t lut_rows;
  const int32_t *ch_slots;
  int32_t x_limit;
  int32_t *x_seen;
  int32_t *x_flags;
  int32_t xcd_split;
  int32_t tchunk;
  uint32_t *sched;
  uint32_t *status;
  int32_t patch_h;
  const int32_t *pred;
};

constexpr int SCHED_Y = 8;
constexpr int SCHED_WORDS = SCHED_Y * 16;
constexpr int SCHED_SLOTS = 64;
constexpr int SCHED_CAPTURE_SLOTS = 960;

struct PatchWalk {
  int64_t first, count, stride;
  int ppb, xcd;
  bool split;
  uint32_t *queue;
  uint32_t *done;
  __device__ __forceinline__ explicit PatchWalk(const ConvMfmaArgs &a) {
    ppb = a.tiles_y * a.tiles_x;
    split = a.xcd_split != 0;
    if (split) {
      xcd = blockIdx.x & 7;
      first = blockIdx.x >> 3;
      stride = gridDim.x >> 3;
      count = (int64_t)((a.B - xcd + 7) >> 3) * ppb;
    } else {
      xcd = 0;
      first = blockIdx.x;
      stride = gridDim.x;
      count = a.npatch;
    }
    queue = a.sched ? a.sched + blockIdx.y * 16 + xcd : nullptr;
    done = a.sched ? a.sched + blockIdx.y * 16 + 8 : nullptr;
  }
  __device__ __forceinline__ int64_t claim() const {
    const int64_t r = stride + (int64_t)atomicAdd(queue, 1u);
    return r < count ? r : count;
  }
  __device__ __forceinline__ void finish(uint32_t processed, int64_t npatch, uint32_t *status) const {
    atomicAdd(done + 1, processed);
    __threadfence();
    const uint32_t total = gridDim.x;
    if (atomicAdd(done, 1u) + 1u == total) {
      __threadfence();
      const uint32_t tally = atomicAdd(done + 1, 0u);
      if (tally != (uint32_t)npatch && status) *(volatile uint32_t *)status = SNNQP_STATUS_QUEUE_CORRUPT;
      for (int i = 0; i < 8; ++i) done[i - 8] = 0u;
      done[1] = 0u;
      __threadfence();
      *done = 0u;
    }
  }
  __device__ __forceinline__ void decode(const ConvMfmaArgs &a, int64_t r, int &b, int &y0,
                                         int &x0) const {
    const int within = (int)(r % ppb);
    const int bi = (int)(r / ppb);
    b = split ? xcd + 8 * bi : bi;
    y0 = (within / a.tiles_x) * a.patch_h;
    x0 = (within % a.tiles_x) * 8;
  }
};

extern "C" __device__ uint32_t snnqp_writelane_i32(uint32_t, uint32_t, uint32_t)
    __asm("llvm.amdgcn.writelane.i32");
__device__ __forceinline__ uint32_t writelane_u32(uint32_t val, int lane, uint32_t old) {
  return snnqp_writelane_i32(val, (uint32_t)lane, old);
}

__device__ __forceinline__ float reset_where(float u, unsigned long long mask) {
  float r;
  asm("v_cndmask_b32_e64 %0, %1, 0, %2" : "=v"(r) : "v"(u), "s"(mask));
  return r;
}

struct LaneConsts {
  float bmean, bmul, bbias, dec;
  float vr;
};

__device__ __forceinline__ uint32_t chan_mask(int cout_base, int Cout) {
  const int valid = Cout - cout_base;
  return valid >= 32 ? 0xFFFFFFFFu : valid <= 0 ? 0u : (1u << valid) - 1u;
}

enum { NF_MUL0 = 1, NF_MUL = 2, NF_DIV = 3, NF_DECAY = 4 };

__host__ inline int neuron_form(const NeuronP &n) {
  if (n.kind == SNNQP_NEURON_LIF) return NF_DECAY;
  if (n.inv_k == 0.0f) return NF_DIV;
  return n.vr == 0.0f ? NF_MUL0 : NF_MUL;
}

__device__ __forceinline__ float lds_read_f32(uint32_t addr) {
  return *(lds_cfloat_t *)(uintptr_t)addr;
}

__device__ __forceinline__ void build_lut(float *lut, int bound, const Dequant &dq,
                                          int tid, int nthreads = 256) {
  for (int i = tid; i <= 2 * bound; i += nthreads) lut[i] = dequant_acc(i - bound, dq);
}

__device__ __forceinline__ int lut_column_start(const uint32_t *scr, int slot) {
  int st = 0;
  for (int k = 0; k < (slot & 3); ++k) st += (int)scr[(slot & ~3) + k];
  return st;
}
__device__ __forceinline__ uint32_t build_lut_channel(float *lut, const uint32_t *scr, int max_rows,
                                                      const Dequant &dq, const BnP &bn, int cout0,
                                                      int Cout, int tid) {
  uint32_t minbits = 0x7F800000u;
  const int c = tid & 127, hf = tid >> 7;
  const int slot = (int)scr[256 + c], col = slot >> 2;
  const int st = lut_column_start(scr, slot);
  const int rows = (int)scr[slot], negx = (int)scr[128 + c];
  if (st + rows > max_rows) return minbits;
  const int co = cout0 + c < Cout ? cout0 + c : Cout - 1;
  float bm = 0.f, bmul = 1.f, bb = 0.f;
  if (bn.mean) { bm = bn.mean[co]; bmul = bn.mul[co]; bb = bn.bias[co]; }
  for (int i = hf; i < rows; i += 2) {
    const float y = bn_apply(dequant_acc(i - negx, dq), bm, bmul, bb);
    lut[(st + i) * 32 + col] = y;
    const uint32_t mag = __float_as_uint(y) & 0x7FFFFFFFu;
    if (mag != 0u && mag < minbits) minbits = mag;
  }
  return minbits;
}

__host__ __device__ __forceinline__ bool lif_fma_is_exact(uint32_t min_x_bits, int j, int T, bool has_u0) {
  if (has_u0 || j < 0) return false;
  const long long e = (long long)j * (T + 1) - 126;
  if (e > 100) return false;
  const uint32_t need = e <= -126 ? 0x00800000u : (uint32_t)(e + 127) << 23;
  return min_x_bits >= need;
}

__device__ __forceinline__ uint32_t lut_bn_min_bits(const float *lut, int bound, const BnP &bn,
                                                    int cout0, int Cout, int tid, int nthreads) {
  int c = cout0 + (tid & 127);
  if (c >= Cout) c = Cout - 1;
  float mean = 0.f, mul = 1.f, bias = 0.f;
  if (bn.mean) { mean = bn.mean[c]; mul = bn.mul[c]; bias = bn.bias[c]; }
  uint32_t mb = 0x7F800000u;
  for (int i = tid >> 7; i <= 2 * bound; i += nthreads >> 7) {
    float x = lut[i] - mean;
    x = x * mul;
    x = x + bias;
    const uint32_t b = __float_as_uint(x) & 0x7FFFFFFFu;
    if (b != 0 && b < mb) mb = b;
  }
  return mb;
}

template <int LUTM, bool OFFS = false>
__device__ __forceinline__ v2f dequant_pair(int a0, int a1, const Dequant &dq, float off = 0.0f) {
  if (LUTM != LUT_NONE) return v2f{lds_read_f32((uint32_t)a0), lds_read_f32((uint32_t)a1)};
  v2f a = {(float)a0, (float)a1};
  if (OFFS) a = a + off;
  const v2f q = fma2(a, v2f{dq.rL, dq.rL}, a * dq.rLlo);
  return q * dq.m;
}

template <int NF, bool FMA = false, bool PACKED = true>
__device__ __forceinline__ v2f neuron_update(v2f x, v2f u, const LaneConsts &lc,
                                             const NeuronP &nrn) {
  if (NF == NF_DECAY) {
    const v2f ud = u * lc.dec;
    return ud + x;
  }
  if (FMA && PACKED) {
    typedef float v2fp __attribute__((ext_vector_type(2)));
    const v2fp up = {u.x, u.y}, xp = {x.x, x.y};
    const v2fp dp = NF == NF_MUL0 ? xp - up : xp - (up - lc.vr);
    const v2fp r = __builtin_elementwise_fma(dp, v2fp{nrn.inv_k, nrn.inv_k}, up);
    return v2f{r.x, r.y};
  }
  const v2f d = NF == NF_MUL0 ? x - u : x - (u - lc.vr);
  if (NF == NF_DIV) return u + v2f{d.x / nrn.k, d.y / nrn.k};
  if (FMA) return fma2(d, v2f{nrn.inv_k, nrn.inv_k}, u);
  const v2f dk = d * nrn.inv_k;
  return u + dk;
}

template <int NF>
__device__ __forceinline__ float neuron_reset(float u, unsigned long long mask,
                                              const LaneConsts &lc) {
  if (NF == NF_MUL0) return reset_where(u, mask);
  float r;
  asm("v_cndmask_b32_e64 %0, %1, %2, %3" : "=v"(r) : "v"(u), "v"(lc.vr), "s"(mask));
  return r;
}

template <int NF, bool BNDONE, bool FMA = false>
__device__ __forceinline__ void neuron_pair(v2f y, float &u0, float &u1,
                                            const LaneConsts &lc, const NeuronP &nrn,
                                            unsigned long long &m0,
                                            unsigned long long &m1) {
  v2f x = y;
  if (!BNDONE) {
    x = x - lc.bmean;
    x = x * lc.bmul;
    x = x + lc.bbias;
  }
  const v2f uu = neuron_update<NF, FMA>(x, v2f{u0, u1}, lc, nrn);
  m0 = __ballot(uu.x >= nrn.vth);
  m1 = __ballot(uu.y >= nrn.vth);
  u0 = neuron_reset<NF>(uu.x, m0, lc);
  u1 = neuron_reset<NF>(uu.y, m1, lc);
}

template <int NF, bool POOL, bool BNDONE, bool FMA = false>
__device__ __forceinline__ uint32_t tile_neurons(const v2f (&y)[8], float (&u)[16],
                                                 const LaneConsts &lc, const NeuronP &nrn) {
  uint32_t myw = 0;
#pragma unroll
  for (int i = 0; i < 16; i += 2) {
    unsigned long long m0, m1;
    neuron_pair<NF, BNDONE, FMA>(y[i >> 1], u[i], u[i + 1], lc, nrn, m0, m1);
    if (POOL) {
      const unsigned long long o = m0 | m1;
      const uint32_t pw = (uint32_t)o | (uint32_t)(o >> 32);
      myw = writelane_u32(pw, i >> 1, myw);
    } else {
      const int r0 = (i & 3) + 8 * (i >> 2);
      myw = writelane_u32((uint32_t)m0, r0, myw);
      myw = writelane_u32((uint32_t)(m0 >> 32), r0 + 4, myw);
      myw = writelane_u32((uint32_t)m1, r0 + 1, myw);
      myw = writelane_u32((uint32_t)(m1 >> 32), r0 + 5, myw);
    }
  }
  return myw;
}

template <int NF, bool POOL, int LUTM, bool FMA = false, bool OFFS = false>
__device__ __forceinline__ uint32_t tile_epilogue(const v16i &acc, float (&u)[16],
                                                  const Dequant &dq,
                                                  const LaneConsts &lc,
                                                  const NeuronP &nrn, int lane,
                                                  float off = 0.0f) {
  v2f y[8];
#pragma unroll
  for (int j = 0; j < 8; ++j) y[j] = dequant_pair<LUTM, OFFS>(acc[2 * j], acc[2 * j + 1], dq, off);
  return tile_neurons<NF, POOL, LUTM == LUT_CHANNEL, FMA>(y, u, lc, nrn);
}

template <int NF, bool POOL, int LUTM, bool FMA = false, bool OFFS = false>
__device__ __forceinline__ uint32_t tile_epilogue_halves(const v16i &acc, float (&u)[16],
                                                         const Dequant &dq, const LaneConsts &lc,
                                                         const NeuronP &nrn, int lane, float off = 0.0f) {
  uint32_t myw = 0;
#pragma unroll
  for (int g = 0; g < 2; ++g) {
    v2f y[4];
#pragma unroll
    for (int j = 0; j < 4; ++j) y[j] = dequant_pair<LUTM, OFFS>(acc[8 * g + 2 * j], acc[8 * g + 2 * j + 1], dq, off);
#pragma unroll
    for (int j = 0; j < 4; ++j) {
      const int i = 8 * g + 2 * j;
      unsigned long long m0, m1;
      neuron_pair<NF, LUTM == LUT_CHANNEL, FMA>(y[j], u[i], u[i + 1], lc, nrn, m0, m1);
      if (POOL) {
        const unsigned long long o = m0 | m1;
        const uint32_t pw = (uint32_t)o | (uint32_t)(o >> 32);
        myw = writelane_u32(pw, i >> 1, myw);
      } else {
        const int r0 = (i & 3) + 8 * (i >> 2);
        myw = writelane_u32((uint32_t)m0, r0, myw);
        myw = writelane_u32((uint32_t)(m0 >> 32), r0 + 4, myw);
        myw = writelane_u32((uint32_t)m1, r0 + 1, myw);
        myw = writelane_u32((uint32_t)(m1 >> 32), r0 + 5, myw);
      }
    }
    __builtin_amdgcn_sched_barrier(0);
  }
  return myw;
}

template <bool POOL>
struct OutStage {
  static constexpr int NPIX = POOL ? 16 : 64;
  static constexpr int FL = POOL ? 32 : 8;
  static constexpr int BYTES = FL * NPIX * 16;
};

template <bool POOL>
__device__ __forceinline__ int out_pix(int tl, int lane) {
  if (POOL) return (tl * 2 + ((lane >> 2) & 1)) * 4 + (lane & 3);
  const int ty = ((lane >> 2) & 1) | (((lane >> 4) & 1) << 1);
  const int tx = (lane & 3) | (((lane >> 3) & 1) << 2);
  return (tl * 4 + ty) * 8 + tx;
}

template <bool POOL, int SLOTS, int NT, int NPIX = OutStage<POOL>::NPIX>
__device__ __forceinline__ void flush_ring(const uint32_t *obuf, const ConvMfmaArgs &a,
                                           int t0, int n, int b, int y0, int x0, int tid) {
  constexpr int PW = POOL ? 4 : 8;
  const int CW = (a.Cout + 31) >> 5;
  const int cwb = blockIdx.y * 4;
  const int nw = min(4, CW - cwb);
  const int OH = POOL ? a.H >> 1 : a.H, OW = POOL ? a.W >> 1 : a.W;
  const int oy0 = POOL ? y0 >> 1 : y0, ox0 = POOL ? x0 >> 1 : x0;
  for (int i = tid; i < n * NPIX; i += NT) {
    const int slot = i / NPIX, pix = i % NPIX;
    const int t = t0 + slot;
    const uint32_t *src = obuf + ((t % SLOTS) * NPIX + pix) * 4;
    const int oy = oy0 + pix / PW, ox = ox0 + pix % PW;
    if (oy >= OH || ox >= OW) continue;
    uint32_t *dst = a.s_out + ((((int64_t)t * a.B + b) * OH + oy) * OW + ox) * CW + cwb;
    if (nw == 4 && (CW & 3) == 0) {
      *(v4i *)dst = *(const v4i *)src;
    } else {
      for (int w = 0; w < nw; ++w) dst[w] = src[w];
    }
  }
}

template <bool POOL>
__device__ __forceinline__ void flush_out(const uint32_t *obuf, const ConvMfmaArgs &a,
                                          int t0, int n, int b, int y0, int x0, int tid) {
  flush_ring<POOL, OutStage<POOL>::FL, 256>(obuf, a, t0, n, b, y0, x0, tid);
}

template <bool LOAD>
__device__ __forceinline__ void u_io_tile(float (&u)[16], const ConvMfmaArgs &a, int b,
                                          int y0, int x0, int cout, int h, int tl) {
  float *uo = a.u_out;
  const float *ui = a.u0;
#pragma unroll
  for (int i = 0; i < 16; ++i) {
    const int y = y0 + tl * 4 + (h | ((i >> 3) << 1));
    const int x = x0 + (i & 7);
    const int64_t o = (((int64_t)b * a.H + y) * a.W + x) * a.Cout + cout;
    const bool in = y < a.H && x < a.W && cout < a.Cout;
    if (LOAD) u[i] = in ? ui[o] : 0.0f;
    else if (in) uo[o] = u[i];
  }
}

template <bool LOAD>
__device__ __forceinline__ void u_io(float (&u)[2][16], const ConvMfmaArgs &a,
                                     int b, int y0, int x0, int cout, int h) {
  float *uo = a.u_out;
  const float *ui = a.u0;
#pragma unroll
  for (int tl = 0; tl < 2; ++tl)
#pragma unroll
    for (int i = 0; i < 16; ++i) {
      const int y = y0 + tl * 4 + (h | ((i >> 3) << 1));
      const int x = x0 + (i & 7);
      const int64_t o = (((int64_t)b * a.H + y) * a.W + x) * a.Cout + cout;
      const bool in = y < a.H && x < a.W && cout < a.Cout;
      if (LOAD) u[tl][i] = in ? ui[o] : 0.0f;
      else if (in) uo[o] = u[tl][i];
    }
}

__device__ __forceinline__ void zero_u(float (&u)[2][16]) {
#pragma unroll
  for (int tl = 0; tl < 2; ++tl)
#pragma unroll
    for (int i = 0; i < 16; ++i) u[tl][i] = 0.0f;
}

__device__ __forceinline__ v16i splat16(int v) {
  return v16i{v, v, v, v, v, v, v, v, v, v, v, v, v, v, v, v};
}

uint32_t *sched_acquire(hipStream_t st, int *dev, int *slot);
void sched_release(int dev, int slot, hipStream_t st);
uint32_t *device_status_word(int dev);

void persistent_limits(const void *kernel, int threads, size_t dyn_lds, int dev, int *cus, int *occ);
int stream_device(hipStream_t st);

template <typename K>
static inline void launch_persistent(K kernel, ConvMfmaArgs a, unsigned gy, hipStream_t st,
                                     size_t dyn_lds = 0, int threads = 256) {
  int dev = 0, cus = 256, occ = 2, slot = -1;
  a.sched = gy <= (unsigned)SCHED_Y ? sched_acquire(st, &dev, &slot) : nullptr;
  if (!a.sched) dev = stream_device(st);
  a.status = a.sched ? device_status_word(dev) : nullptr;
  persistent_limits((const void *)kernel, threads, dyn_lds, dev, &cus, &occ);
  const int64_t gmax = (int64_t)cus * occ;
  unsigned gx = (unsigned)(a.npatch < gmax ? a.npatch : gmax);
  a.xcd_split = 0;
  if (gx >= 64 && a.B >= 8) {
    gx &= ~7u;
    a.xcd_split = 1;
  }
  hipLaunchKernelGGL(kernel, dim3(gx, gy), dim3(threads), dyn_lds, st, a);
  if (a.sched) sched_release(dev, slot, st);
}

enum { DQ_ARITH = 1, DQ_ONE = 2, DQ_TABLE = 3 };
constexpr int DQT_MAXA = 2047;
void launch_conv3x3_bits(const ConvMfmaArgs &a, int cin_walk, bool i8, int nf, bool pool, int dq,
                         bool fma, bool bnf, unsigned gy, hipStream_t st);
bool conv_k16_enabled();

}
```

snnquantprune_amd/csrc/kernels.h:

```cpp
#pragma once
#include "common.h"
#include "tile_util.h"

namespace snnqp {

struct GenericDepth {
  int32_t D, KD, OD, stride, pad_lo, in_dil, k_dil;
};
int run_generic(const void *x, int in_type, int64_t xs_t, int64_t xs_b, int32_t T,
                int32_t B, const snnqp_conv_geom_t *g, const snnqp_weight_t *w,
                const snnqp_bn_t *bn, const snnqp_neuron_t *nrn, const float *u0,
                float *u_out, void *s_out, int s_type, int32_t *acc_out,
                hipStream_t st, int pool = 1, const int32_t *pred = nullptr,
                const GenericDepth *dz = nullptr);

const char *conv3x3_mfma_unsupported(int in_type, const snnqp_conv_geom_t *g,
                                     const snnqp_weight_t *w, const int8_t *wt,
                                     const snnqp_neuron_t *nrn, int s_type);
const char *conv3x3_currents_unsupported(int in_type, int64_t NB, const snnqp_conv_geom_t *g,
                                         const snnqp_weight_t *w, const int8_t *wt);
int run_conv3x3_currents(const void *x, int64_t NB, const snnqp_conv_geom_t *g,
                         const snnqp_weight_t *w, const int8_t *wt, float *y, int32_t *acc,
                         hipStream_t st);
int run_current_min(const snnqp_weight_t *w, const snnqp_bn_t *bn, int32_t bound, int32_t Cout,
                    uint32_t *out_bits, hipStream_t st);
int conv3x3_bits_dequant_form(const snnqp_weight_t *w, const snnqp_neuron_t *nrn);
int run_conv3x3_mfma(const void *x, int in_type, int64_t xs_t, int64_t xs_b,
                     int32_t T, int32_t B, const snnqp_conv_geom_t *g,
                     const snnqp_weight_t *w, const int8_t *wt,
                     const snnqp_bn_t *bn, const snnqp_neuron_t *nrn,
                     const float *u0, float *u_out, uint32_t *s_out, int pool,
                     int x_max, int32_t *x_seen, int32_t *x_flags, hipStream_t st,
                     const int32_t *pred = nullptr);

uint32_t *device_status_word(int dev);
int zero_words_async(uint32_t *p, int64_t nwords, hipStream_t st);
uint32_t device_status_read(int dev);
int refuse_after_device_report(hipStream_t st, const char *who);
const char *device_status_text(uint32_t code);
bool dq_table_trusted(int dev, hipStream_t st);
void check_code_bound_once(int dev, const int8_t *w, int64_t K, int32_t N, int32_t bound, hipStream_t st);
int64_t dq_table_fallbacks(bool reset);
int stream_device(hipStream_t st);

const char *fseq_gemm_unsupported(int in_type, const snnqp_conv_geom_t *g,
                                  const snnqp_weight_t *w);
int run_fseq_gemm(const void *x, int in_type, int64_t NB, const snnqp_conv_geom_t *g,
                  const snnqp_weight_t *w, float *y, hipStream_t st);

const char *dense_mfma_unsupported(int in_type, int32_t K, int32_t N,
                                   const snnqp_weight_t *w, const int8_t *wt,
                                   const snnqp_neuron_t *nrn, int s_type);
int run_dense_mfma(const void *x, int in_type, int64_t xs_t, int64_t xs_b, int32_t T, int32_t B,
                   int32_t K, int32_t N, const snnqp_weight_t *w, const int8_t *wt,
                   const snnqp_bn_t *bn, const snnqp_neuron_t *nrn, const float *u0,
                   float *u_out, uint32_t *s_out, hipStream_t st);

const char *dense_wide_unsupported(int in_type, int32_t T, int32_t K, int32_t N, int64_t xs_t,
                                   int64_t xs_b, const void *x, const snnqp_weight_t *w,
                                   const int8_t *wt, const snnqp_neuron_t *nrn, int s_type);
int run_dense_wide(const void *x, int in_type, int64_t xs_t, int64_t xs_b, int32_t T, int32_t B,
                   int32_t K, int32_t N, const snnqp_weight_t *w, const int8_t *wt,
                   const snnqp_bn_t *bn, const snnqp_neuron_t *nrn, const float *u0,
                   float *u_out, uint32_t *s_out, int32_t *x_flags, hipStream_t st);

const char *conv_gated_unsupported(const snnqp_conv_geom_t *g, const snnqp_weight_t *w);
const char *dense_gated_unsupported(int32_t HW, int32_t C, int32_t N, const snnqp_weight_t *w);

int run_dense_fp6(const void *x, int64_t xs_t, int64_t xs_b, int32_t T, int32_t B, int32_t K,
                  int32_t N, const snnqp_weight_t *w, const snnqp_bn_t *bn,
                  const snnqp_neuron_t *nrn, const float *u0, float *u_out, uint32_t *s_out,
                  int row_tiles, void *ws, int64_t ws_bytes, hipStream_t st);
int64_t dense_fp6_workspace_bytes(int32_t T, int32_t B, int32_t K, int32_t N);

}
```

snnquantprune_amd/linen.py:

```python

from __future__ import annotations

import dataclasses
import functools
import hashlib
import math
import threading
from collections.abc import MutableMapping
from typing import Any, Callable, Dict, Iterable, Optional, Sequence

import torch

_tls = threading.local()


def _stack():
  if not hasattr(_tls, "stack"):
    _tls.stack = []
  return _tls.stack


class ConfigDict(MutableMapping):

  def __init__(self, *args, **kwargs):
# ... 14 lines not shown

  def __iter__(self):
    return iter(self._d)

  def __len__(self):
    return len(self._d)

  def __contains__(self, k):
    return k in self._d

  def __getattr__(self, k):
    try:
      return self._d[k]
    except KeyError:
      raise AttributeError(k)

  def __setattr__(self, k, v):
    self[k] = v

  def __delattr__(self, k):
    del self._d[k]

  def __hash__(self):
    return id(self)

  def __eq__(self, other):
    return self is other

  def __repr__(self):
    return "ConfigDict(%r)" % (self._d,)

  def to_dict(self):
    return {k: (v.to_dict() if isinstance(v, ConfigDict) else v)
            for k, v in self._d.items()}


FrozenConfigDict = ConfigDict



_DTYPE_POLICY = "strict"
_dtype_warned = False


def set_compute_dtype_policy(policy: str):
  global _DTYPE_POLICY
  if policy not in ("strict", "float32"):
    raise ValueError("compute dtype policy must be 'strict' or 'float32'")
  _DTYPE_POLICY = policy


_CHANNEL_COMPACTION = True


def set_channel_compaction(enabled: bool):
  global _CHANNEL_COMPACTION
  _CHANNEL_COMPACTION = bool(enabled)


def channel_compaction() -> bool:
  return _CHANNEL_COMPACTION


_CONV_KPACK = True


def set_conv_kpack(enabled: bool):
  global _CONV_KPACK
  _CONV_KPACK = bool(enabled)


def conv_kpack() -> bool:
  return _CONV_KPACK


def set_conv_k16(enabled: bool):
  from . import _lib
  _lib.lib().snnqp_set_conv_k16(1 if enabled else 0)


def conv_k16() -> bool:
  from . import _lib
  return bool(_lib.lib().snnqp_set_conv_k16(-1))


_TRAIN_CONV_MFMA = True


def set_train_conv_mfma(enabled: bool) -> bool:
  global _TRAIN_CONV_MFMA
  old = _TRAIN_CONV_MFMA
  _TRAIN_CONV_MFMA = bool(enabled)
  return old


def train_conv_mfma() -> bool:
  return _TRAIN_CONV_MFMA


def check_compute_dtype(dtype, who: str):
  global _dtype_warned
  if dtype in (torch.float32, None, "float32"):
    return
  if _DTYPE_POLICY == "float32":
    if not _dtype_warned:
      import sys
      print("snnquantprune_amd: %s asked for %r; computing in float32 (nn.set_compute_dtype_policy)"
            % (who, dtype), file=sys.stderr)
      _dtype_warned = True
    return
  raise NotImplementedError(
      "%s computes in float32 (got %r); nn.set_compute_dtype_policy('float32') runs such a "
      "request in float32 instead of refusing it" % (who, dtype))




def _default_device():
  return torch.device("cuda") if torch.cuda.is_available() else torch.device("cpu")


def zeros(key, shape, dtype=torch.float32):
  return torch.zeros(tuple(shape), dtype=dtype, device=_default_device())


def ones(key, shape, dtype=torch.float32):
  return torch.ones(tuple(shape), dtype=dtype, device=_default_device())


def constant(value):
  def init(key, shape, dtype=torch.float32):
    return torch.full(tuple(shape), float(value), dtype=dtype, device=_default_device())
  return init


def lecun_normal():
  def init(key, shape, dtype=torch.float32):
    shape = tuple(shape)
    fan_in = 1
    for d in shape[:-1]:
      fan_in *= d
    std = math.sqrt(1.0 / max(fan_in, 1)) / 0.87962566103423978
    w = torch.empty(shape, dtype=torch.float32)
    torch.nn.init.trunc_normal_(w, mean=0.0, std=std, a=-2 * std, b=2 * std,
                                generator=key)
    return w.to(dtype).to(_default_device())
  return init


class Variable:
  def __init__(self, module, col, name):
    self._m, self._col, self._name = module, col, name

  @property
  def value(self):
    return self._m._get(self._col, self._name)

  @value.setter
  def value(self, v):
    root = self._m._root
    if not (root.initializing or self._col in root.mutable):
      raise RuntimeError("collection %r is immutable" % self._col)
    self._m._set(self._col, self._name, v)


class _Root:
# ... 390 lines not shown
```

snnquantprune_amd/ops.py:

```python

from __future__ import annotations

import ctypes
from dataclasses import dataclass
from typing import Optional, Sequence, Tuple

import torch

from . import _lib as L




class PackedSpikes:

  def __init__(self, bits: torch.Tensor, channels: int):
    assert bits.dtype == torch.int32 and bits.is_contiguous()
    assert bits.shape[-1] == (channels + 31) // 32
    self.bits = bits
    self.channels = int(channels)
    self.flat_perm = None
    self.chan_map = None

  @property
# ... 212 lines not shown
    frames *= d
  data = torch.empty(lead + (frame_units(H, W, fmt),),
                     dtype=torch.int32 if fmt == L.EV1 else torch.uint8, device=x.device)
  L.check(L.lib().snnqp_pack_frames(_ptr(x), frames, H, W, fmt, _ptr(data), _ptr(flags), _stream()))
  return PackedFrames(data, H, W, fmt)


def pack_frames_checked(x: torch.Tensor) -> Tuple[PackedFrames, torch.Tensor]:
  _require_gpu(x)
  assert x.dtype in (torch.uint8, torch.float32) and x.shape[-1] == 2 and x.ndim >= 3, (x.dtype, tuple(x.shape))
  x = x.contiguous()
  H, W = x.shape[-3], x.shape[-2]
  lead = tuple(x.shape[:-3])
  frames = 1
  for d in lead:
    frames *= d
  data = torch.empty(lead + (frame_units(H, W, L.EV1),), dtype=torch.int32, device=x.device)
  flags = torch.empty(1, dtype=torch.int32, device=x.device)
  L.check(L.lib().snnqp_pack_frames_checked(_ptr(x), L.U8 if x.dtype == torch.uint8 else L.F32, frames, H, W,
                                            _ptr(data), _ptr(flags), _stream()))
  return PackedFrames(data, H, W, L.EV1), flags


def unpack_frames(p: PackedFrames) -> torch.Tensor:
  _require_gpu(p.data)
  lead = tuple(p.data.shape[:-1])
  frames = 1
  for d in lead:
    frames *= d
  y = torch.empty(lead + (p.H, p.W, 2), dtype=torch.uint8, device=p.device)
  L.check(L.lib().snnqp_unpack_frames(_ptr(p.data), p.fmt, frames, p.H, p.W, _ptr(y), _stream()))
  return y




def _stream():
  return ctypes.c_void_p(torch.cuda.current_stream().cuda_stream)


def _ptr(t: Optional[torch.Tensor]):
  return None if t is None else ctypes.c_void_p(t.data_ptr())


def _require_gpu(*ts):
  for t in ts:
    if t is None:
      continue
    if not t.is_cuda:
      raise RuntimeError(
          "snnquantprune_amd ops run on the GPU only (tensor on %s); there is no "
          "CPU fallback" % t.device)


def _f32c(t: torch.Tensor) -> torch.Tensor:
  if t.dtype != torch.float32:
    t = t.to(torch.float32)
  return t.contiguous()


def is_pow2(x: float) -> bool:
  import math
  if not (x > 0) or math.isinf(x):
    return False
  m, _ = math.frexp(x)
  return m == 0.5


@dataclass
class Weight:
  wtype: int
  w: torch.Tensor
  L: float = 1.0
  m: float = 1.0
  wt: Optional[torch.Tensor] = None
  abs_sum_max: int = 0
  code_max: int = 0
  min_current_bits: int = 0
  col_sum: Optional[torch.Tensor] = None
  wt6: Optional[torch.Tensor] = None
  ch_stack_max: int = 0
  ch_slots: Optional[torch.Tensor] = None
  wt_cin: int = 0

  def struct(self) -> L.WeightT:
    st = self.__dict__.get("_cstruct")
    if st is None:
      st = L.WeightT(self.wtype, self.w.data_ptr(), float(self.L), float(self.m),
                     int(self.abs_sum_max), int(self.code_max),
                     None if self.col_sum is None else self.col_sum.data_ptr(),
                     None if self.wt6 is None else self.wt6.data_ptr(),
                     int(self.min_current_bits), int(self.ch_stack_max),
                     None if self.ch_slots is None else self.ch_slots.data_ptr(), int(self.wt_cin))
      self.__dict__["_cstruct"] = st
    return st

  @property
  def is_int(self):
    return self.wtype == L.W_I8


@dataclass
class Neuron:
  kind: int
  k: float = 2.0
  v_threshold: float = 1.0
  v_reset: float = 0.0
  decay: Optional[torch.Tensor] = None

  def struct(self) -> L.NeuronT:
    return L.NeuronT(self.kind, float(self.k), float(self.v_threshold),
                     float(self.v_reset),
                     None if self.decay is None else self.decay.data_ptr())


@dataclass
class BnCoeffs:
  mean: torch.Tensor
  mul: torch.Tensor
  bias: torch.Tensor
  flags: int = 0

  def struct(self) -> L.BnT:
    return L.BnT(self.mean.data_ptr(), self.mul.data_ptr(), self.bias.data_ptr(), int(self.flags))


@dataclass
class ConvGeom:
  H: int
  W: int
  Cin: int
  Cout: int
  KH: int
  KW: int
  stride: Tuple[int, int] = (1, 1)
  pad: Tuple[Tuple[int, int], Tuple[int, int]] = ((0, 0), (0, 0))
  in_dil: Tuple[int, int] = (1, 1)
  k_dil: Tuple[int, int] = (1, 1)
  groups: int = 1

  def struct(self) -> L.ConvGeomT:
    return L.ConvGeomT(self.H, self.W, self.Cin, self.Cout, self.KH, self.KW,
                       self.stride[0], self.stride[1], self.pad[0][0],
                       self.pad[0][1], self.pad[1][0], self.pad[1][1],
                       self.in_dil[0], self.in_dil[1], self.k_dil[0],
                       self.k_dil[1], self.groups)

  def tag(self) -> str:
    return "%dx%dx%d->%d" % (self.H, self.W, self.Cin, self.Cout)

  def out_hw(self) -> Tuple[int, int]:
    oh, ow = ctypes.c_int32(), ctypes.c_int32()
    g = self.struct()
    L.check(L.lib().snnqp_conv_out_shape(ctypes.byref(g), ctypes.byref(oh),
                                         ctypes.byref(ow)))
    return oh.value, ow.value


@dataclass(frozen=True)
class Conv3dGeom:
  D: int
  H: int
  W: int
  Cin: int
  Cout: int
  KD: int
  KH: int
  KW: int
  stride: Tuple[int, int, int] = (1, 1, 1)
  pad: Tuple[Tuple[int, int], Tuple[int, int], Tuple[int, int]] = ((0, 0), (0, 0), (0, 0))
  in_dil: Tuple[int, int, int] = (1, 1, 1)
  k_dil: Tuple[int, int, int] = (1, 1, 1)
  groups: int = 1

  def struct(self) -> L.Conv3dGeomT:
    i3 = ctypes.c_int32 * 3
# ... 400 lines not shown


def current_min_bits(weight: Weight, bn: Optional[BnCoeffs], bound: int, cout: int) -> int:
  global _current_min_cache
  if _current_min_cache is None:
    from ._cache import TensorCache
    _current_min_cache = TensorCache(64)
  key = (weight.w,) + ((bn.mean, bn.mul, bn.bias) if bn is not None else (None, None, None))
  extra = (int(bound), int(cout), float(weight.L), float(weight.m))
  v = _current_min_cache.get(key, extra)
  if v is None:
    _require_gpu(weight.w)
    out = torch.full((1,), 0x7F800000, dtype=torch.int32, device=weight.w.device)
    w = weight.struct()
    b = bn.struct() if bn is not None else None
    L.check(L.lib().snnqp_current_min(ctypes.byref(w), ctypes.byref(b) if b is not None else None,
                                      int(bound), int(cout), _ptr(out), _stream()))
    v = int(out.item()) & 0xFFFFFFFF
    _current_min_cache.put(key, extra, v)
  return v


def _tb_strides(x, T, B, time_major: bool, unit: int):
  if time_major:
    return B * unit, unit
  return unit, T * unit


def _zero_step_carry(u_out: Optional[torch.Tensor], u0: Optional[torch.Tensor], T: int):
  if u_out is not None and T == 0:
    if u0 is None:
      u_out.zero_()
    else:
      u_out.copy_(u0)


def conv_lif_forward(x, geom: ConvGeom, weight: Weight, neuron: Neuron,
                     bn: Optional[BnCoeffs] = None, u0: Optional[torch.Tensor] = None,
                     want_u: bool = True, packed_out: bool = False, pool: int = 1,
                     impl: int = L.IMPL_AUTO, time_major: bool = True, x_max: int = 0,
                     x_seen: Optional[torch.Tensor] = None,
                     fallback: Optional[FloatFallback] = None, binary_first: bool = False,
                     logical: Optional[Tuple[int, int, int]] = None):
  xt, in_type = _in_desc(x)
  xt = xt.contiguous()
  _require_gpu(xt, weight.w, u0)
  x_flags = None
  if in_type == L.F32 and weight.is_int:
    if fallback is None:
      raise ValueError("float32 input into integer codes needs a FloatFallback (the float32 kernel)")
    x_flags = torch.empty(1, dtype=torch.int32, device=xt.device)
  if x_seen is not None:
    assert x_seen.dtype == torch.int32 and x_seen.numel() >= 8 and x_seen.is_cuda, \
        "x_seen: eight int32 device words (snnqp.h)"
  T, B = (xt.shape[0], xt.shape[1]) if time_major else (xt.shape[1], xt.shape[0])
  if isinstance(x, PackedFrames):
    assert (x.H, x.W, 2) == (geom.H, geom.W, geom.Cin) and xt.ndim == 3, (x.shape, geom)
    unit = xt.shape[-1]
  else:
    unit = geom.H * geom.W * (xt.shape[-1])
  xs_t, xs_b = _tb_strides(xt, T, B, time_major, unit)
  OH, OW = geom.out_hw()
  dev = xt.device
  u_out = torch.empty((B, OH, OW, geom.Cout), dtype=torch.float32, device=dev) \
      if want_u else None
  if u0 is not None:
    u0 = _f32c(u0)
    assert tuple(u0.shape) == (B, OH, OW, geom.Cout), (u0.shape, (B, OH, OW, geom.Cout))
  _zero_step_carry(u_out, u0, T)
  oshape = (T, B, OH // pool, OW // pool)
  if packed_out:
    s = torch.empty(oshape + ((geom.Cout + 31) // 32,), dtype=torch.int32, device=dev)
  else:
    s = torch.empty(oshape + (geom.Cout,), dtype=torch.float32, device=dev)
  g, w, n = geom.struct(), weight.struct(), neuron.struct()
  b = bn.struct() if bn is not None else None
  cin_l, cout_l = (geom.Cin, geom.Cout) if logical is None else logical[:2]
  tag = "conv%dx%d[%dx%dx%d->%d]" % (geom.KH, geom.KW, geom.H, geom.W, cin_l, cout_l)
  if _PROFILE is not None and in_type == L.BITS and weight.is_int and "dequant" not in PROFILE_NOTES.get(tag, {}):
    PROFILE_NOTES.setdefault(tag, {})["dequant"] = conv_dequant_form(weight, neuron)
  if _PROFILE is not None and logical is not None:
    PROFILE_NOTES.setdefault(tag, {})["channels"] = {
        "cin": geom.Cin, "cout": geom.Cout, "live_out": int(logical[2])}
  speculate = (binary_first and packed_out and not isinstance(x, (PackedFrames, PackedSpikes))
               and in_type in (L.U8, L.F32) and geom.Cin == 2 and weight.is_int and impl != L.IMPL_GENERIC
               and xt.ndim == 5)
  with _timed(tag):
    if speculate:
      pf, not_binary = pack_frames_checked(xt)
      ps_t, ps_b = _tb_strides(pf.data, T, B, time_major, pf.data.shape[-1])
      try:
        L.check(L.lib().snnqp_conv_lif_forward(
            _ptr(pf.data), L.EV1, ps_t, ps_b, T, B, ctypes.byref(g), ctypes.byref(w),
            _ptr(weight.wt), ctypes.byref(b) if b is not None else None, ctypes.byref(n),
            _ptr(u0), _ptr(u_out), _ptr(s), L.BITS, pool, impl, 1, None, None, _stream()))
      except L.SnnqpError as e:
        if e.code != L.EUNSUPPORTED:
          raise
        speculate = False
    if speculate:
      L.check(L.lib().snnqp_conv_lif_forward_pred(
          _ptr(not_binary), _ptr(xt), in_type, xs_t, xs_b, T, B, ctypes.byref(g), ctypes.byref(w),
          _ptr(weight.wt), ctypes.byref(b) if b is not None else None, ctypes.byref(n),
          _ptr(u0), _ptr(u_out), _ptr(s), L.BITS, pool,
          int(x_max), _ptr(x_seen), _ptr(x_flags), _stream()))
    else:
      L.check(L.lib().snnqp_conv_lif_forward(
          _ptr(xt), in_type, xs_t, xs_b, T, B, ctypes.byref(g), ctypes.byref(w),
          _ptr(weight.wt), ctypes.byref(b) if b is not None else None, ctypes.byref(n),
          _ptr(u0), _ptr(u_out), _ptr(s), L.BITS if packed_out else L.F32, pool, impl,
          int(x_max), _ptr(x_seen), _ptr(x_flags), _stream()))
  if fallback is not None:
    xf = _f32c(xt if fallback.x is None else fallback.x)
    pred = x_flags if fallback.pred is None else fallback.pred
    fw = fallback.weight.struct()
    fs_t, fs_b = _tb_strides(xf, T, B, time_major, geom.H * geom.W * geom.Cin)
    L.check(L.lib().snnqp_conv_lif_forward_if(
        _ptr(pred), _ptr(xf), L.F32, fs_t, fs_b, T, B, ctypes.byref(g), ctypes.byref(fw),
        ctypes.byref(b) if b is not None else None, ctypes.byref(n), _ptr(u0), _ptr(u_out), _ptr(s),
        L.BITS if packed_out else L.F32, pool, _stream()))
  return u_out, (PackedSpikes(s, geom.Cout) if packed_out else s)


def dense_lif_forward(x, weight: Weight, K: int, N: int, neuron: Neuron,
                      bn: Optional[BnCoeffs] = None, u0: Optional[torch.Tensor] = None,
                      want_u: bool = True, packed_out: bool = False,
                      impl: int = L.IMPL_AUTO, time_major: bool = True,
                      fallback: Optional[FloatFallback] = None):
  xt, in_type = _in_desc(x)
  xt = xt.contiguous()
  _require_gpu(xt, weight.w, u0)
  x_flags = None
  if in_type == L.F32 and weight.is_int:
    if fallback is None:
      raise ValueError("float32 rows into integer codes need a FloatFallback (the float32 kernel)")
    x_flags = torch.empty(1, dtype=torch.int32, device=xt.device)
  T, B = (xt.shape[0], xt.shape[1]) if time_major else (xt.shape[1], xt.shape[0])
  xs_t, xs_b = _tb_strides(xt, T, B, time_major, xt.shape[-1])
  dev = xt.device
  u_out = torch.empty((B, N), dtype=torch.float32, device=dev) if want_u else None
  if u0 is not None:
    u0 = _f32c(u0)
    assert tuple(u0.shape) == (B, N)
  _zero_step_carry(u_out, u0, T)
  if packed_out:
    s = torch.empty((T, B, (N + 31) // 32), dtype=torch.int32, device=dev)
  else:
    s = torch.empty((T, B, N), dtype=torch.float32, device=dev)
  w, n = weight.struct(), neuron.struct()
  b = bn.struct() if bn is not None else None
  ws = _dense_workspace(dev, int(L.lib().snnqp_dense_workspace_bytes(in_type, T, B, K, N, ctypes.byref(w)))) \
      if (packed_out and impl != L.IMPL_GENERIC) else None
  with _timed("dense[%d->%d]" % (K, N)):
    L.check(L.lib().snnqp_dense_lif_forward_ws(
        _ptr(xt), in_type, xs_t, xs_b, T, B, K, N, ctypes.byref(w), _ptr(weight.wt),
        ctypes.byref(b) if b is not None else None, ctypes.byref(n), _ptr(u0),
        _ptr(u_out), _ptr(s), L.BITS if packed_out else L.F32, impl, _ptr(x_flags),
        _ptr(ws), 0 if ws is None else ws.numel(), _stream()))
  if fallback is not None:
    xf = _f32c(xt if fallback.x is None else fallback.x)
    pred = x_flags if fallback.pred is None else fallback.pred
    fw = fallback.weight.struct()
    L.check(L.lib().snnqp_dense_lif_forward_if(
        _ptr(pred), _ptr(xf), L.F32, xs_t, xs_b, T, B, K, N, ctypes.byref(fw),
        ctypes.byref(b) if b is not None else None, ctypes.byref(n), _ptr(u0), _ptr(u_out), _ptr(s),
        L.BITS if packed_out else L.F32, _stream()))
# ... 26 lines not shown
  xt, in_type = _in_desc(x)
  xt = xt.contiguous()
  _require_gpu(xt, w1.w, w2.w)
  T, B = (xt.shape[0], xt.shape[1]) if time_major else (xt.shape[1], xt.shape[0])
  xs_t, xs_b = _tb_strides(xt, T, B, time_major, xt.shape[-1])
  dev = xt.device
  if N2 % group:
    raise ValueError("vote: %d features not divisible by group %d" % (N2, group))
  logits = torch.empty((B, N2 // group), dtype=torch.float32, device=dev)
  x_flags = None
  if in_type == L.F32:
    if fallback is None or fallback.x is not None:
      raise ValueError("float32 rows into the fused head need a FloatFallback of the first block")
    x_flags = torch.empty(1, dtype=torch.int32, device=dev)
  elif fallback is not None:
    raise ValueError("a FloatFallback goes with float32 rows; uint8 / bit-packed rows have nothing to redo")
  redo = in_type == L.F32
  s1 = torch.empty((T, B, (N1 + 31) // 32), dtype=torch.int32, device=dev) if (want_s1 or redo) else None
  s2 = torch.empty((T, B, (N2 + 31) // 32), dtype=torch.int32, device=dev) if (want_s2 or redo) else None
  a, b, n1, n2 = w1.struct(), w2.struct(), nrn1.struct(), nrn2.struct()
  nws = _head_ws_bytes.get((T, B, N1))
  if nws is None:
    nws = _head_ws_bytes[(T, B, N1)] = int(L.lib().snnqp_dense_head_workspace_bytes(T, B, N1))
  ws = _dense_workspace(dev, nws)
  with _timed("dense_head[%d->%d->%d]" % (K, N1, N2)):
    L.check(L.lib().snnqp_dense_head_forward(
        _ptr(xt), in_type, xs_t, xs_b, T, B, K, N1, ctypes.byref(a), _ptr(w1.wt), ctypes.byref(n1),
        N2, ctypes.byref(b), _ptr(w2.wt), ctypes.byref(n2), int(group),
        _ptr(s1) if (want_s1 or redo) else None, _ptr(s2) if (want_s2 or redo) else None,
        _ptr(logits), _ptr(x_flags), _ptr(ws), 0 if ws is None else ws.numel(), _stream()))
  if redo:
    fw = fallback.weight.struct()
    lib = L.lib()
    L.check(lib.snnqp_dense_lif_forward_if(_ptr(x_flags), _ptr(xt), L.F32, xs_t, xs_b, T, B, K, N1,
                                           ctypes.byref(fw), None, ctypes.byref(n1), None, None, _ptr(s1),
                                           L.BITS, _stream()))
    cw1 = (N1 + 31) // 32
    L.check(lib.snnqp_dense_lif_forward_if(_ptr(x_flags), _ptr(s1), L.BITS, B * cw1, cw1, T, B, N1, N2,
                                           ctypes.byref(b), None, ctypes.byref(n2), None, None, _ptr(s2),
                                           L.BITS, _stream()))
    L.check(lib.snnqp_vote_if(_ptr(x_flags), _ptr(s2), L.BITS, T, B, N2, int(group), _ptr(logits), _stream()))
  return (logits, PackedSpikes(s1, N1) if want_s1 else None,
          PackedSpikes(s2, N2) if want_s2 else None)


_head_ws_bytes = {}


def fallback_counts(reset: bool = False) -> dict:
  conv, dense = ctypes.c_int64(), ctypes.c_int64()
  buf = ctypes.create_string_buffer(256)
  L.check(L.lib().snnqp_fallback_counts(ctypes.byref(conv), ctypes.byref(dense), buf, 256,
                                        1 if reset else 0))
  return {"conv_blocks": conv.value, "dense_blocks": dense.value,
          "last_reason": buf.value.decode("utf-8", "replace")}


def device_status(device=None, reset: bool = False) -> int:
  dev = torch.cuda.current_device() if device is None else torch.device(device).index
  code = ctypes.c_uint32()
  L.check(L.lib().snnqp_device_status(int(dev or 0), ctypes.byref(code), 1 if reset else 0))
  return int(code.value)


def workqueue_stats(reset: bool = False) -> dict:
  a, b, c = ctypes.c_int64(), ctypes.c_int64(), ctypes.c_int64()
  L.check(L.lib().snnqp_workqueue_stats(ctypes.byref(a), ctypes.byref(b), ctypes.byref(c), 1 if reset else 0))
  return {"captured_static_walks": a.value, "busy_static_walks": b.value, "dequant_table_fallbacks": c.value}


def workqueue_capture_mark(device) -> int:
  m = ctypes.c_int64()
  L.check(L.lib().snnqp_workqueue_capture_mark(int(torch.device(device).index or 0), ctypes.byref(m)))
  return int(m.value)


def workqueue_capture_release(device, begin: int, end: int):
  L.check(L.lib().snnqp_workqueue_capture_release(int(torch.device(device).index or 0), int(begin), int(end)))


DQ_FORMS = {1: "arith", 2: "one", 3: "table"}


def conv_dequant_form(w: Weight, nrn: Neuron) -> str:
  ws, ns = w.struct(), nrn.struct()
  rc = L.lib().snnqp_conv_dequant_form(ctypes.byref(ws), ctypes.byref(ns))
  if rc < 0:
    L.check(rc)
  return DQ_FORMS[rc]




def lif_forward(x: torch.Tensor, neuron: Neuron, bn: Optional[BnCoeffs] = None,
                u0: Optional[torch.Tensor] = None, want_u: bool = True,
                packed_out: bool = False):
  x = _f32c(x)
  _require_gpu(x, u0)
  T, C = x.shape[0], x.shape[-1]
  R = (x.numel() // (T * C)) if T * C else 0
  u_out = torch.empty(x.shape[1:], dtype=torch.float32, device=x.device) if want_u else None
  if u0 is not None:
    u0 = _f32c(u0)
    assert tuple(u0.shape) == tuple(x.shape[1:])
  _zero_step_carry(u_out, u0, T)
  if packed_out:
    s = torch.empty(tuple(x.shape[:-1]) + ((C + 31) // 32,), dtype=torch.int32,
                    device=x.device)
  else:
    s = torch.empty_like(x)
  n = neuron.struct()
  b = bn.struct() if bn is not None else None
  L.check(L.lib().snnqp_lif_forward(
      _ptr(x), T, R, C, ctypes.byref(b) if b is not None else None, ctypes.byref(n),
      _ptr(u0), _ptr(u_out), _ptr(s), L.BITS if packed_out else L.F32, _stream()))
  return u_out, (PackedSpikes(s, C) if packed_out else s)


def batchnorm_forward(x: torch.Tensor, bn: BnCoeffs) -> torch.Tensor:
  x = _f32c(x)
  _require_gpu(x)
  C = x.shape[-1]
  y = torch.empty_like(x)
  b = bn.struct()
  L.check(L.lib().snnqp_batchnorm_forward(_ptr(x), x.numel() // C if C else 0, C,
                                          ctypes.byref(b), _ptr(y), _stream()))
  return y


def maxpool2x2(x):
  if isinstance(x, PackedSpikes):
    bits = x.bits
    _require_gpu(bits)
    H, W = bits.shape[-3], bits.shape[-2]
    lead = tuple(bits.shape[:-3])
    NB = 1
    for d in lead:
      NB *= d
    y = torch.empty(lead + (H // 2, W // 2, bits.shape[-1]), dtype=torch.int32,
                    device=bits.device)
    L.check(L.lib().snnqp_maxpool2x2(_ptr(bits), L.BITS, NB, H, W, x.channels, _ptr(y),
                                     _stream()))
    return PackedSpikes(y, x.channels)
  x = _f32c(x)
  _require_gpu(x)
  H, W, C = x.shape[-3:]
  lead = tuple(x.shape[:-3])
  NB = 1
  for d in lead:
    NB *= d
  y = torch.empty(lead + (H // 2, W // 2, C), dtype=torch.float32, device=x.device)
  L.check(L.lib().snnqp_maxpool2x2(_ptr(x), L.F32, NB, H, W, C, _ptr(y), _stream()))
  return y


def spatial_mean(x) -> torch.Tensor:
  if isinstance(x, PackedSpikes):
    t, typ, C = x.bits, L.BITS, x.channels
  else:
    t, typ, C = _f32c(x), L.F32, x.shape[-1]
  _require_gpu(t)
  lead = tuple(t.shape[:-3])
  HW = t.shape[-3] * t.shape[-2]
  NB = 1
  for d in lead:
    NB *= d
# ... 202 lines not shown
```

snnquantprune_amd/packing.py:

```python

from __future__ import annotations

from typing import Optional

import torch

from . import _lib as L
from . import linen as _nn
from . import ops
from ._cache import TensorCache
from .quant import QuantDesc

AUTO_INTEGER_INPUTS = True


class _Speculate:

  def __bool__(self):
    return True

  def __repr__(self):
    return "SPECULATE"


SPECULATE = _Speculate()


import contextlib


@contextlib.contextmanager
def integer_inputs(enabled: bool):
  global AUTO_INTEGER_INPUTS
  old, AUTO_INTEGER_INPUTS = AUTO_INTEGER_INPUTS, enabled
  try:
    yield
  finally:
    AUTO_INTEGER_INPUTS = old


def table_slots(ranges):
  import numpy as np
  r = np.asarray(ranges, np.int64)
  n128 = (r.size + 127) // 128 * 128
  r = np.concatenate([r, np.zeros(n128 - r.size, np.int64)])
  slots = np.zeros(n128, np.int32)
  worst = 0
  for g in range(n128 // 128):
    col = np.zeros(32, np.int64)
    for w in range(4):
      ch = 128 * g + 32 * w + np.argsort(-r[128 * g + 32 * w:128 * g + 32 * w + 32], kind="stable")
      banks = np.argsort(col, kind="stable")
      slots[ch] = 4 * banks + w
      col[banks] += r[ch]
    worst = max(worst, int(col.max()))
  return slots, worst


def _int_weight_of(codes: torch.Tensor, Lq: float, m: float) -> ops.Weight:
  c2 = codes.reshape(-1, codes.shape[-1]).to(torch.int32)
  side = torch.maximum(c2.clamp(min=0).sum(0).max(), (-c2).clamp(min=0).sum(0).max())
  stats = torch.stack([side, c2.abs().max()]).tolist()
  col = c2.sum(0).to(torch.int32).contiguous() if codes.ndim == 2 else None
  slots, stack = None, 0
  if codes.ndim == 4 and codes.shape[2] == 2:
    slots, stack = table_slots(c2.abs().sum(0).cpu().numpy())
    slots = torch.from_numpy(slots).to(codes.device)
  return ops.Weight(L.W_I8, codes, Lq, m, abs_sum_max=int(stats[0]),
                    code_max=int(stats[1]), col_sum=col, ch_stack_max=stack, ch_slots=slots)


def conv_cin_pad(cin: int, kpack: bool = True) -> int:
  if not 0 < cin <= 128:
    raise ValueError("bit-input conv blocks take 1 to 128 input channels")
  if kpack:
    return (cin + 31) // 32 * 32
  return 64 if cin <= 64 else 128


class PackedKernel:
  def __init__(self, kernel: torch.Tensor, desc: Optional[QuantDesc],
               mask: Optional[torch.Tensor]):
    self.kernel = kernel
    self.desc = desc
    self.mask = mask
    self._int = None
    self._int_done = False
    self._float = None
    self._wt = {}

  def int_weight(self) -> Optional[ops.Weight]:
    if self._int_done:
      return self._int
    self._int_done = True
    d = self.desc
    if d is None or d.bits > 8:
      return None
    _, codes, flags = ops.quantize(d.kind, self.kernel, self.mask, d.bits, d.p0, d.p1,
                                   want_fq=False, want_codes=True, sign=d.sign)
    if int(flags.item()) & (L.FLAG_CODE_OVERFLOW | L.FLAG_MASK_NOT_BINARY):
      return None
    self._int = _int_weight_of(codes, d.L, d.m)
    return self._int

  def sliced(self, rows, cols) -> "PackedKernel":
    base = self.int_weight()
    assert base is not None, "only integer codes are sliced"
    import numpy as np
    key = ("_sliced", None if rows is None else np.asarray(rows).tobytes(),
           None if cols is None else np.asarray(cols).tobytes())
    pk = self._wt.get(key)
    if pk is None:
      codes = base.w
      dev = codes.device
      if rows is not None:
        codes = codes.index_select(codes.ndim - 2, torch.as_tensor(np.asarray(rows), device=dev))
      if cols is not None:
        codes = codes.index_select(codes.ndim - 1, torch.as_tensor(np.asarray(cols), device=dev))
      pk = self._wt[key] = _SlicedKernel(codes.contiguous(), self.desc, base)
    return pk

  def host_codes(self):
    if "_host" not in self._wt:
      self._wt["_host"] = self.int_weight().w.cpu().numpy().astype("int64")
    return self._wt["_host"]

  def gated_codes(self):
    w = self.int_weight()
    if w is None or self.kernel.ndim != 4 or tuple(self.kernel.shape[:2]) != (3, 3) or not (0 < w.code_max <= 127):
      return None
    if "_gated" not in self._wt:
      self._wt["_gated"] = ops.pack_codes_gated(w.w, w.code_max)
    return self._wt["_gated"]

  def gated_dense_codes(self, C: int, HW: int):
    w = self.int_weight()
    if (w is None or self.kernel.ndim != 2 or self.kernel.shape[0] != C * HW or not (0 < w.code_max <= 127)
        or HW > 16 or C not in (32, 64, 96, 128)):
      return None
    key = ("_dgated", C, HW)
    if key not in self._wt:
      self._wt[key] = ops.pack_codes_dense_gated(w.w, C, HW, w.code_max)
    return self._wt[key]

  def float_weight(self) -> ops.Weight:
    if self._float is None:
      d = self.desc
      k = self.kernel.to(torch.float32).contiguous()
      if d is not None:
        fq, _, _ = ops.quantize(d.kind, k, self.mask, d.bits, d.p0, d.p1,
                                want_fq=True, want_codes=False, sign=d.sign)
      elif self.mask is not None:
        fq = k * self.mask.to(k.device, torch.float32)
      else:
        fq = k
      self._float = ops.Weight(L.W_F32, fq.contiguous())
    return self._float

  def int_weight_mfma(self, n_pad: int, row_perm: Optional[torch.Tensor] = None,
                            perm_key=None) -> Optional[ops.Weight]:
    base = self.int_weight()
    if base is None:
      return None
    kpack = _nn.conv_kpack()
    key = (n_pad, perm_key, kpack)
    w = self._wt.get(key)
    if w is None:
      codes = base.w.reshape(-1, base.w.shape[-1])
      if row_perm is not None:
        codes = codes.index_select(0, row_perm)
      codes = codes.contiguous()
      wt_cin = 0
      if self.kernel.ndim == 2 and codes.shape[0] % 32:
        pad = 32 - codes.shape[0] % 32
        tiles_src = torch.cat([codes, codes.new_zeros((pad, codes.shape[1]))], 0)
      elif (self.kernel.ndim == 4 and row_perm is None and (0 if kpack else 2) < base.w.shape[2] <= 128
            and base.w.shape[2] % (32 if kpack else 64)):
        kh, kw, ci, co = base.w.shape
        cpad = conv_cin_pad(ci, kpack)
        padded = base.w.new_zeros((kh, kw, cpad, co))
        padded[:, :, :ci] = base.w
        tiles_src = padded.reshape(-1, co)
        wt_cin = cpad
      else:
        tiles_src = codes
      wt = ops.pack_codes_mfma(tiles_src, n_pad) if tiles_src.shape[0] % 32 == 0 else None
      wt6 = None
      if self.kernel.ndim == 2 and 0 < base.code_max <= 7:
        wt6 = ops.pack_codes_fp6(codes, n_pad)
      w = ops.Weight(L.W_I8, codes, base.L, base.m, wt=wt, abs_sum_max=base.abs_sum_max,
                     code_max=base.code_max, col_sum=base.col_sum, wt6=wt6, ch_stack_max=base.ch_stack_max,
                     ch_slots=base.ch_slots, wt_cin=wt_cin)
      self._wt[key] = w
    return w


class _SlicedKernel(PackedKernel):

  def __init__(self, codes: torch.Tensor, desc, base: ops.Weight):
    super().__init__(codes, desc, None)
    self._int = _int_weight_of(codes, base.L, base.m)
    self._int_done = True

  def float_weight(self):
    raise RuntimeError("a sliced kernel has integer codes only")


_cache = TensorCache(128)


def get_packed(kernel, desc, mask) -> PackedKernel:
  pk = _cache.get((kernel, mask), desc)
  if pk is None:
    pk = _cache.put((kernel, mask), desc, PackedKernel(kernel, desc, mask))
  return pk


def clear_cache():
  _cache.clear()


def prepare_input(x, prefer_bits: Optional[bool] = None):
  if isinstance(x, (ops.PackedSpikes, ops.PackedFrames)):
    return x, True
  if isinstance(x, ops.GatedSpikes):
    return x, False
  if not isinstance(x, torch.Tensor):
    x = torch.as_tensor(x)
  if x.dtype in (torch.uint8, torch.bool):
    return (x if x.dtype == torch.uint8 else x.to(torch.uint8)), True
  if x.dtype != torch.float32:
    x = x.to(torch.float32)
  if not AUTO_INTEGER_INPUTS or x.numel() == 0:
    return x, False
  return x, SPECULATE
```

snnquantprune_amd/prune_utils.py:

```python

from __future__ import annotations

import numpy as np
import torch


def check_quant_obj(x) -> bool:
  return isinstance(x, dict) and "kernel" in x


def _map_layers(fn, tree):
  if check_quant_obj(tree):
    return fn(tree)
  if isinstance(tree, dict):
    return {k: _map_layers(fn, v) for k, v in tree.items()}
  return tree


def _layers(tree, out=None):
  out = [] if out is None else out
  if check_quant_obj(tree):
    out.append(tree)
  elif isinstance(tree, dict):
    for v in tree.values():
# ... 66 lines not shown

def _np(a):
  if a is None:
    return None
  if isinstance(a, torch.Tensor):
    return a.detach().cpu().numpy()
  return np.asarray(a)


def _current_f32(acc, L, m, bn):
  f = np.float32
  y = (acc.astype(f) / f(L)) * f(m)
  if bn is not None:
    mean, mul, bias = bn
    y = ((y - mean.astype(f)) * mul.astype(f)) + bias.astype(f)
  return y.astype(f)


def _neuron_factor(neuron):
  from . import _lib as L
  kind = getattr(neuron, "kind", None)
  vth, vr = float(np.float32(neuron.v_threshold)), float(np.float32(neuron.v_reset))
  if kind == L.NEURON_MULTI_STEP_LIF:
    tau = float(np.float32(neuron.k))
    if not tau >= 1.0:
      return None
    k = 1.0 / tau
  elif kind == L.NEURON_PARAMETRIC_LEAKY_IF:
    k = float(np.float32(neuron.k))
    if not 0.0 < k <= 1.0:
      return None
  else:
    return None
  if k < _K_MIN:
    return None
  return k, vth, vr


def channel_liveness(kernel_codes, dequant, bn, neuron, x_max, live_in=None, u0=None):
  codes = _np(kernel_codes)
  live = np.ones(codes.shape[-1], bool)
  if dequant is None:
    return live
  nf = _neuron_factor(neuron)
  if nf is None or u0 is not None:
    return live
  k, vth, vr = nf
  if not vth > 0.0:
    return live
  c = codes.reshape((-1,) + codes.shape[-2:]).astype(np.int64)
  if live_in is not None:
    li = np.asarray(_np(live_in), bool)
    assert li.shape == (c.shape[1],), (li.shape, c.shape)
    c = c * li[None, :, None]
  pos = np.clip(c, 0, None).sum((0, 1))
  neg = np.clip(-c, 0, None).sum((0, 1))
  if isinstance(bn, (tuple, list)) or bn is None:
    bnn = None if bn is None else tuple(_np(v).astype(np.float32) for v in bn)
  else:
    bnn = (_np(bn.mean).astype(np.float32), _np(bn.mul).astype(np.float32),
           _np(bn.bias).astype(np.float32))
  L_, m_ = dequant
  xm = int(x_max)
  e1 = _current_f32(pos * xm, L_, m_, bnn).astype(np.float64)
  e0 = _current_f32(-neg * xm, L_, m_, bnn).astype(np.float64)
  x_hi, x_lo = np.maximum(e0, e1), np.minimum(e0, e1)
  fin = np.isfinite(x_hi) & np.isfinite(x_lo)
  bound = np.maximum(0.0, x_hi + vr)
  S = np.maximum(np.abs(x_hi), np.abs(x_lo)) + abs(vr)
  slack = (32.0 * _EPS32 * S + 8.0 * _ETA32) / k
  silent = fin & (bound + slack + 2.0 * _ETA32 < vth)
  return ~silent


def computed_channels(live, multiple: int = 32):
  live = np.asarray(live, bool)
  idx = np.flatnonzero(live)
  n = max(multiple, -(-idx.size // multiple) * multiple)
  n = min(n, live.size)
  pad = np.flatnonzero(~live)[:n - idx.size]
  return np.concatenate([idx, pad]).astype(np.int64)


def _host_codes(leaf, bits):
  f = np.float32
  w = _np(leaf["kernel"]).astype(f)
  a = f(_np(leaf["DuQ_0"]["a"]).reshape(-1)[0])
  c = f(_np(leaf["DuQ_0"]["c"]).reshape(-1)[0])
  if a == f(-1) or bits == -1 or bits > 8:
    return None
  L_ = f(2 ** (bits - 1) - 1)
  q = np.rint(np.clip(w / a, f(-1), f(1)) * L_)
  if "prune_0" in leaf:
    q = q * _np(leaf["prune_0"]["mask"]).astype(f)
  return q.astype(np.int64), (float(L_), float(c))


def _host_bn(params, stats, name, eps=1e-5):
  f = np.float32
  mean = _np(stats[name]["mean"]).astype(f)
  var = _np(stats[name]["var"]).astype(f)
  mul = f(1) / np.sqrt(var + f(eps))
  if "scale" in params[name]:
    mul = mul * _np(params[name]["scale"]).astype(f)
  bias = _np(params[name]["bias"]).astype(f) if "bias" in params[name] else np.zeros_like(mean)
  return mean, mul.astype(f), bias


def conv_net_liveness(variables, config, x_max, nblocks: int = 3, neuron=None):
  from . import _lib as L
  from . import ops
  params, stats = variables["params"], variables.get("batch_stats", {})
  if neuron is None:
    nd = config.neuron_dynamics
    kw = dict(getattr(nd, "keywords", {}) or {})
    neuron = ops.Neuron(L.NEURON_MULTI_STEP_LIF, float(np.float32(kw.get("tau", 2.0))),
                        float(kw.get("v_threshold", 1.0)), float(kw.get("v_reset", 0.0)))
  q = config.quant
  out, live_in, xm = [], None, int(x_max)
  for i in range(nblocks):
    bits = int(q.layer_bits[i]) if ("layer_bits" in q and q.layer_bits is not None) else q.bits
    hc = _host_codes(params["QuantConv_%d" % i], bits) if "weight" in q else None
    if hc is None:
      live = np.ones(_np(params["QuantConv_%d" % i]["kernel"]).shape[-1], bool)
    else:
      live = channel_liveness(hc[0], hc[1], _host_bn(params, stats, "BatchNorm_%d" % i), neuron,
                              xm, live_in)
    out.append(live)
    live_in, xm = live, 1
  return out
```

snnquantprune_amd/spiking_learning.py:

```python

from __future__ import annotations

import dataclasses
import math
from typing import Any, Callable, Optional

import numpy as np

import torch

from . import _lib as L
from . import linen as nn
from . import ops
from . import packing
from ._cache import TensorCache
from .flax_qconv import QuantConv
from .flax_qdense import QuantDense

Array = Any




def uniform(scale=1e-2, dtype=torch.float32):
# ... 231 lines not shown
  def __call__(self, u, inputs):
    if self.pool not in (1, 2):
      raise ValueError("pool must be 1 or 2")
    if self._fusable():
      return self._fused(u, inputs)
    return self._composed(u, ops.expand_channels(inputs))

  @staticmethod
  def _input_bound(x):
    if isinstance(x, ops.PackedFrames):
      return 1 if x.fmt == L.EV1 else 15
    if isinstance(x, ops.PackedSpikes):
      return 1
    if isinstance(x, torch.Tensor) and x.dtype == torch.uint8:
      return 255
    return None

  def _channel_plan(self, pk, nrn, bn, x_max, cmap_in):
    from . import prune_utils
    w = pk.int_weight()
    full_in = w.w.shape[-2]
    live_in = None
    if cmap_in is not None:
      live_in = np.zeros(full_in, bool)
      live_in[cmap_in.index[cmap_in.live]] = True
    key = (w.w,) + ((bn.mean, bn.mul, bn.bias) if bn is not None else (None, None, None))
    extra = (int(x_max), None if live_in is None else live_in.tobytes(), nrn.kind, float(nrn.k),
             float(nrn.v_threshold), float(nrn.v_reset))
    plan = _plan_cache.get(key, extra)
    if plan is None:
      bnh = None if bn is None else (bn.mean.cpu().numpy(), bn.mul.cpu().numpy(), bn.bias.cpu().numpy())
      live = prune_utils.channel_liveness(pk.host_codes(), (w.L, w.m), bnh, nrn, x_max, live_in)
      idx = prune_utils.computed_channels(live)
      plan = _plan_cache.put(key, extra, (ops.ChannelMap(idx, live[idx], live.size),)
                             if idx.size < live.size else (None,))
    return plan[0]

  def _fused(self, u, inputs):
    conn, norm = self.connection_fn, self.norm_fn
    if isinstance(inputs, ops.GatedSpikes):
      out = self._gated_block(u, inputs)
      if out is not None:
        return out
      inputs = inputs.to_dense()
    if isinstance(conn, QuantConv) and len(conn._ksize()) == 3:
      return self._conv3d_block(u, inputs)
    flat = getattr(inputs, "flat_perm", None)
    x, integer = packing.prepare_input(inputs)
    spec = integer is packing.SPECULATE
    if flat is not None:
      x.flat_perm = flat
    u0 = None if (u is None or isinstance(u, ZeroCarry)) else u
    tm = not self.batch_major_input
    is_dense = isinstance(conn, QuantDense)
    cmap_in = getattr(x, "chan_map", None)
    if cmap_in is not None:
      full_cin = cmap_in.full if flat is None else cmap_in.full * flat[1] * flat[2]
      pk = conn.packed_kernel(full_cin)
      if not (integer and pk.int_weight() is not None and is_dense == (flat is not None)
              and (is_dense or len(conn._ksize()) == 2)):
        x = ops.expand_channels(x)
        flat = x.flat_perm
        cmap_in = None
      elif not is_dense:
        x, cmap_in = ops.truncate_silent_channels(x)
    cin = x.shape[-1]
    pk = conn.packed_kernel(cin if cmap_in is None else full_cin)
    packed_out = bool(integer) if self.packed is None else bool(self.packed)
    rows = None
    if cmap_in is not None:
      rows = cmap_in.index
      if flat is not None:
        hw = flat[1] * flat[2]
        rows = (rows[:, None] * hw + np.arange(hw)[None, :]).reshape(-1)
    cmap_out = None
    x_bound = self._input_bound(x)
    if (self.compact and nn.channel_compaction() and not is_dense and integer is True and u0 is None
        and not self.return_state and packed_out and len(conn._ksize()) == 2 and x_bound is not None
        and self.impl != L.IMPL_GENERIC and pk.int_weight() is not None):
      cmap_out = self._channel_plan(pk, self.neural_dynamics.neuron(conn.features),
                                    self.norm_fn.coeffs(conn.features) if self.norm_fn is not None else None,
                                    x_bound, cmap_in)
    if rows is not None or cmap_out is not None:
      pk = pk.sliced(rows, None if cmap_out is None else cmap_out.index)
    w = None
    if integer:
      if is_dense:
        n_pad = (conn.features + 31) // 32 * 32
        perm = None
        if flat is not None:
          perm = _flat_perm(*flat, device=pk.kernel.device)
        w = pk.int_weight_mfma(n_pad, perm, perm_key=flat)
        flat = None if w is not None else flat
      else:
        w = pk.int_weight_mfma((conn.features + 31) // 32 * 32)
    if w is None:
      w = pk.float_weight()
      spec = False
    fb = None
    if spec:
      fbw = pk.float_weight()
      T_ = x.shape[0] if tm else x.shape[1]
      if is_dense:
        B_ = x.shape[1] if tm else x.shape[0]
        xs_t, xs_b = (B_ * cin, cin) if tm else (cin, T_ * cin)
        direct = (x.ndim == 3 and w.wt is not None and w.col_sum is not None and cin % 16 == 0
                  and cin <= 65536 and conn.features > 128 and T_ <= 64 and self.impl == L.IMPL_AUTO
                  and packed_out and (x.data_ptr() & 15) == 0 and x.is_contiguous()
                  and (max(T_ - 1, 0) * xs_t + 128 * xs_b + cin) * 4 < (1 << 31))
      else:
        direct = (x.ndim == 5 and self.impl != L.IMPL_GENERIC and packed_out
                  and self._event_layer_geometry(conn.geometry(tuple(x.shape[2:-1]), cin)))
      x_f32 = x

      def narrowed():
        if not is_dense and cin >= 32:
          xn, pred = ops.pack_bits_checked(x_f32)
        else:
          xn, pred = ops.narrow_f32_async(x_f32)
        return xn, ops.FloatFallback(fbw, x=x_f32, pred=pred)
      if direct:
        fb = ops.FloatFallback(fbw)
      else:
        x, fb = narrowed()
        spec = False
    if flat is not None:
      c, h, ww = flat
      d = x.to_dense() if isinstance(x, ops.PackedSpikes) else x.to(torch.float32)
      d = d.reshape(d.shape[0], d.shape[1], h, ww, c).permute(0, 1, 4, 2, 3)
      x = d.reshape(d.shape[0], d.shape[1], c * h * ww).contiguous()
    nrn = self.neural_dynamics.neuron(conn.features)
    bn = norm.coeffs(conn.features) if norm is not None else None
    if cmap_out is not None and bn is not None:
      bn = _sliced_bn(bn, cmap_out)

    if isinstance(x, ops.PackedFrames):
      direct = (not is_dense and w.wtype == L.W_I8 and packed_out
                and self.impl != L.IMPL_GENERIC and x.ndim == 5
                and self._event_layer_geometry(conn.geometry(tuple(x.shape[2:-1]), cin)))
      if not direct:
        x = ops.unpack_frames(x)

    if w.wtype == L.W_F32 and self.impl == L.IMPL_AUTO and (
        isinstance(x, ops.PackedSpikes) or x.dtype in (torch.float32, torch.uint8)):
      geom = None
      if is_dense and x.ndim == 3:
        geom = ops.ConvGeom(1, 1, cin, conn.features, 1, 1)
      elif not is_dense and len(conn._ksize()) == 2 and x.ndim == 5:
        geom = conn.geometry(tuple(x.shape[2:-1]), cin)
      if geom is not None and ops.fseq_gemm_supported(geom):
        if self.pool == 2 and is_dense:
          raise ValueError("pool=2 needs a convolutional block")
        return self._float_block(x, tm, is_dense, geom, w, nrn, bn, u0, packed_out)

    if is_dense:
      if x.ndim != 3:
        raise ValueError("QuantDense block expects [T, B, K] inputs, got %s" % (x.shape,))
      try:
        u_out, s = ops.dense_lif_forward(x, w, cin, conn.features, nrn, bn=bn, u0=u0,
                                         want_u=self.return_state, packed_out=packed_out,
                                         impl=self.impl, time_major=tm, fallback=fb)
      except L.SnnqpError as e:
        if e.code != L.EUNSUPPORTED or not spec:
          raise
        x, fb = narrowed()
        u_out, s = ops.dense_lif_forward(x, w, cin, conn.features, nrn, bn=bn, u0=u0,
                                         want_u=self.return_state, packed_out=packed_out,
# ... 271 lines not shown
```

Before: 96130 samples/s.

## Pack the last half-filled output-channel group of the first conv into one MFMA

When channel compaction leaves the final 32-channel wave of the 2-input first conv layer with only 16 live channels, the wave now processes two pixel rows per MFMA. The upper 16 lanes reuse the lower 16 channels' weights shifted by a row, so that wave does half the MFMA work, and channels beyond cout_fire are masked out. This adds a cout_fire field to the weight descriptor, a HALF kernel variant, a shared planning helper and a query API. It also widens the per-channel lookup table ranges for the duplicated group. The change adds template instantiations and ABI surface, and it only applies to event-bit input with a single chunk and per-channel tables.

```diff
diff --git a/include/snnqp.h b/include/snnqp.h
--- a/include/snnqp.h
+++ b/include/snnqp.h
@@ -61,6 +61,7 @@
   int32_t ch_stack_max;
   const int32_t *ch_slots;
   int32_t wt_cin;
+  int32_t cout_fire;
 } snnqp_weight_t;
 
 #define SNNQP_BN_MEAN_ZERO 1
@@ -107,6 +108,9 @@
 const char *snnqp_build_flags(void);
 
 int snnqp_set_conv_k16(int enabled);
+int snnqp_set_event_half_group(int enabled);
+int snnqp_conv_event_half_group(int in_type, int32_t T, const snnqp_conv_geom_t *g, const snnqp_weight_t *w,
+                                const snnqp_neuron_t *nrn, int has_state, int pool, int x_max);
 
 int snnqp_conv_out_shape(const snnqp_conv_geom_t *g, int32_t *OH, int32_t *OW);
 
diff --git a/snnquantprune_amd/_lib.py b/snnquantprune_amd/_lib.py
--- a/snnquantprune_amd/_lib.py
+++ b/snnquantprune_amd/_lib.py
@@ -27,7 +27,7 @@
   _fields_ = [("wtype", c_int32), ("w", c_void_p), ("L", c_float), ("m", c_float),
               ("abs_sum_max", c_int32), ("code_max", c_int32), ("col_sum", c_void_p),
               ("wt_fp6", c_void_p), ("min_current_bits", c_uint32), ("ch_stack_max", c_int32),
-              ("ch_slots", c_void_p), ("wt_cin", c_int32)]
+              ("ch_slots", c_void_p), ("wt_cin", c_int32), ("cout_fire", c_int32)]
 
 
 BN_MEAN_ZERO, BN_BIAS_ZERO, BN_MUL_UNIFORM = 1, 2, 4
@@ -60,6 +60,9 @@
     "snnqp_last_error": (c_char_p, []),
     "snnqp_build_flags": (c_char_p, []),
     "snnqp_set_conv_k16": (c_int, [c_int]),
+    "snnqp_set_event_half_group": (c_int, [c_int]),
+    "snnqp_conv_event_half_group": (c_int, [c_int, c_int32, POINTER(ConvGeomT), POINTER(WeightT),
+                                            POINTER(NeuronT), c_int, c_int, c_int]),
     "snnqp_conv_out_shape": (c_int, [POINTER(ConvGeomT), POINTER(c_int32),
                                      POINTER(c_int32)]),
     "snnqp_quantize": (c_int, [c_int, c_void_p, c_void_p, c_int64, c_int, c_float,
diff --git a/snnquantprune_amd/csrc/api.hip b/snnquantprune_amd/csrc/api.hip
--- a/snnquantprune_amd/csrc/api.hip
+++ b/snnquantprune_amd/csrc/api.hip
@@ -6,6 +6,8 @@
 
 static std::atomic<int> g_conv_k16{1};
 bool conv_k16_enabled() { return g_conv_k16.load(std::memory_order_relaxed) != 0; }
+static std::atomic<int> g_event_half_group{1};
+bool event_half_group_enabled() { return g_event_half_group.load(std::memory_order_relaxed) != 0; }
 
 static thread_local std::string g_last_error;
 
@@ -36,6 +38,11 @@
   return snnqp::g_conv_k16.exchange(enabled ? 1 : 0, std::memory_order_relaxed);
 }
 
+int snnqp_set_event_half_group(int enabled) {
+  if (enabled < 0) return snnqp::event_half_group_enabled() ? 1 : 0;
+  return snnqp::g_event_half_group.exchange(enabled ? 1 : 0, std::memory_order_relaxed);
+}
+
 int snnqp_conv_out_shape(const snnqp_conv_geom_t *g, int32_t *OH, int32_t *OW) {
   SNNQP_REQUIRE(g && OH && OW, SNNQP_EINVAL, "conv_out_shape: null argument");
   SNNQP_REQUIRE(g->stride_h > 0 && g->stride_w > 0 && g->in_dil_h > 0 &&
diff --git a/snnquantprune_amd/csrc/blocks.hip b/snnquantprune_amd/csrc/blocks.hip
--- a/snnquantprune_amd/csrc/blocks.hip
+++ b/snnquantprune_amd/csrc/blocks.hip
@@ -63,6 +63,13 @@
   SNNQP_REQUIRE(w && nrn, SNNQP_EINVAL, "conv_dequant_form: null descriptor");
   SNNQP_REQUIRE(w->wtype == SNNQP_W_I8, SNNQP_EINVAL, "conv_dequant_form: int8 codes only");
   return conv3x3_bits_dequant_form(w, nrn);
+}
+
+int snnqp_conv_event_half_group(int in_type, int32_t T, const snnqp_conv_geom_t *g, const snnqp_weight_t *w,
+                                const snnqp_neuron_t *nrn, int has_state, int pool, int x_max) {
+  SNNQP_REQUIRE(g && w && nrn, SNNQP_EINVAL, "conv_event_half_group: null descriptor");
+  SNNQP_CHECK_NEURON_KIND(nrn, "conv_event_half_group");
+  return conv3x3_event_half_group(in_type, T, g, w, nrn, has_state != 0, pool, x_max);
 }
 
 int snnqp_conv_lif_forward(const void *x, int in_type, int64_t x_stride_t,
diff --git a/snnquantprune_amd/csrc/conv3x3_u8c2.hip b/snnquantprune_amd/csrc/conv3x3_u8c2.hip
--- a/snnquantprune_amd/csrc/conv3x3_u8c2.hip
+++ b/snnquantprune_amd/csrc/conv3x3_u8c2.hip
@@ -42,11 +42,13 @@
   if (IN == SNNQP_EV1) return SNNQP_U8C2_EV1_WPS;
   return ONE ? SNNQP_U8C2_ONE_WPS : U8C2_WPS;
 }
-template <int NF, bool POOL, int LUTM, int IN = SNNQP_U8, bool ONE = false>
+template <int NF, bool POOL, int LUTM, int IN = SNNQP_U8, bool ONE = false, bool HALF = false>
 __global__ void __launch_bounds__(256, (u8c2_waves<NF, POOL, LUTM, IN, ONE>()))
 conv3x3_u8c2_kernel(ConvMfmaArgs a) {
   constexpr int FL = OutStage<POOL>::FL;
   constexpr bool EV1 = IN == SNNQP_EV1;
+  static_assert(!HALF || (EV1 && ONE && LUTM == LUT_CHANNEL && NF == NF_MUL0),
+                "the half group: bit-packed frames, one chunk, per-channel tables, NF_MUL0");
   constexpr bool EV4 = IN == SNNQP_EV4;
   constexpr bool F32IN = IN == SNNQP_F32;
   static_assert(TCHUNK % FL == 0, "flush period must divide the staging chunk");
@@ -64,7 +66,9 @@
   const bool wave_on = cout_base < a.Cout;
   const int cout = wave_on ? cout_base + n : n;
   const int cpar = cout < a.Cout ? cout : a.Cout - 1;
-  const uint32_t cmask = chan_mask(cout_base, a.Cout);
+  const uint32_t cmask = chan_mask(cout_base, a.cout_fire);
+  const bool half_wave = HALF && cout_base + 32 == a.Cout;
+  const int ctab = half_wave && n >= 16 ? cout - 16 : cout;
   uint32_t *wgw = obuf + OutStage<POOL>::BYTES / 4;
   if (tid == 0) { wgw[0] = 0x7F800000u; wgw[1] = 0u; }
   typedef int v2i_a8 __attribute__((ext_vector_type(2)));
@@ -93,7 +97,7 @@
     for (int j = 0; j < 16; ++j) {
       const int k = 16 * h + j, dy = k >> 3, b = k & 7;
       if (k < 24 && b < 6 && wave_on && cout < a.Cout) {
-        const int code = a.w[(int64_t)(6 * dy + b) * a.Cout + cout];
+        const int code = a.w[(int64_t)(6 * dy + b) * a.Cout + ctab];
         pos += code > 0 ? code : 0;
         neg += code < 0 ? -code : 0;
       }
@@ -116,8 +120,8 @@
     for (int k = 0; k < 4; ++k) total += (int)scr[(slot & ~3) + k];
     ch_row0 = start + neg * a.x_limit;
     if (total > a.lut_rows && a.status) *(volatile uint32_t *)a.status = SNNQP_STATUS_BOUND;
-    const uint32_t mb = build_lut_channel((float *)(lds + lut_off), scr, a.lut_rows, a.dq, a.bn,
-                                          blockIdx.y * 128, a.Cout, tid);
+    const uint32_t mb = build_lut_channel<HALF>((float *)(lds + lut_off), scr, a.lut_rows, a.dq, a.bn,
+                                                blockIdx.y * 128, a.Cout, tid);
     atomicMin(wgw, mb);
     lds_barrier();
   }
@@ -127,12 +131,14 @@
   }
 
   float acc_off = 0.0f;
+  int tab0 = 0;
   v4i bf, bfg;
   {
     int bias = 0;
     if (LUTM == LUT_SHARED) bias = (int)lds_addr(lds) + lut_off + 4 * a.lut_bound;
     if (LUTM == LUT_CHANNEL)
       bias = (int)lds_addr(lds) + lut_off + 4 * (ch_row0 * 32 + ch_col);
+    if (HALF) tab0 = bias;
     int q = bias / 127;
     const int r = bias - 127 * q;
     int wsum = 0;
@@ -144,7 +150,11 @@
       for (int j = 0; j < 4; ++j) {
         const int k = 16 * h + 4 * d + j;
         uint32_t bv = 0, bg = 0;
-        if (k < 24) {
+        if (HALF && half_wave) {
+          const int kk = n >= 16 ? k - 8 : k;
+          if (kk >= 0 && kk < 24 && (kk & 7) < 6)
+            bv = (uint8_t)(a.w[(int64_t)(6 * (kk >> 3) + (kk & 7)) * a.Cout + ctab] * 8);
+        } else if (k < 24) {
           const int dy = k >> 3, b = k & 7;
           if (b < 6 && cout < a.Cout) {
             const int code = a.w[(int64_t)(6 * dy + b) * a.Cout + cout];
@@ -178,16 +188,18 @@
   const int tx = (n & 3) | (((n >> 3) & 1) << 2);
   const int cpy = tx & 1;
   const int px0 = (int)lds_addr(lds) + cpy * HCOPY2 + 2 * tx + 2 * cpy;
+  const int tyh = half_wave ? 2 * ty : ty;
   int offA[2], offB[2];
 #pragma unroll
   for (int tl = 0; tl < 2; ++tl) {
-    offA[tl] = px0 + (ty + 4 * tl + (h ? 2 : 0)) * HROW2;
+    offA[tl] = px0 + (tyh + 4 * tl + (h ? 2 : 0)) * HROW2;
     offB[tl] = h ? (int)lds_addr(lds) + HCONST2 : px0 + (ty + 4 * tl + 1) * HROW2;
   }
+  if (HALF && half_wave) offB[1] = tab0;
   const uint8_t *xb = (const uint8_t *)a.x;
-  const int ob0 = out_pix<POOL>(0, lane) * 4 + wave;
+  const int ob0 = (half_wave ? lane : out_pix<POOL>(0, lane)) * 4 + wave;
   const int ob1 = out_pix<POOL>(1, lane) * 4 + wave;
-  const bool store_lane = POOL ? lane < 8 : lane < 32;
+  const bool store_lane = POOL ? lane < (half_wave ? 16 : 8) : (half_wave || lane < 32);
   uint32_t seen = 0;
   uint32_t hist[6] = {0, 0, 0, 0, 0, 0};
   const int s_pix = tid & 127;
@@ -358,6 +370,34 @@
       constexpr bool FMA = decltype(fma_tag)::value;
       constexpr bool OFFS = MODE == LUT_NONE;
       const v4i bw = OFFS ? bfg : bf;
+      if constexpr (HALF) {
+        if (half_wave) {
+          int ctab0 = offB[1];
+          asm volatile("" : "+v"(ctab0));
+          const v16i c0 = splat16(ctab0);
+          for (int tf = 0; tf < nt; tf += FL) {
+            const int nf = min(FL, nt - tf);
+#pragma unroll 1
+            for (int tt = tf; tt < tf + nf; ++tt) {
+              const uint32_t img = (uint32_t)(tt * HIMG2);
+              const v2i_a4 lo = *(lds_cv2i_t *)(uintptr_t)(img + (uint32_t)offA[0]);
+              const v2i_a4 hi = *(lds_cv2i_t *)(uintptr_t)(img + (uint32_t)offA[0] + (uint32_t)HROW2);
+              const v16i acc = __builtin_amdgcn_mfma_i32_32x32x32_i8(v4i{lo.x, lo.y, hi.x, hi.y}, bw, c0,
+                                                                     0, 0, 0);
+              const uint32_t word = tile_epilogue_halves<NF, POOL, MODE, FMA, OFFS, true>(
+                  acc, u[0], a.dq, lc, a.nrn, lane, acc_off);
+              if (store_lane) {
+                uint32_t *o = obuf + ((t0 + tt) % FL) * (OutStage<POOL>::NPIX * 4);
+                o[ob0] = word & cmask;
+              }
+            }
+            lds_barrier();
+            flush_out<POOL>(obuf, a, t0 + tf, nf, b, y0, x0, tid);
+            lds_barrier();
+          }
+          return;
+        }
+      }
       for (int tf = 0; tf < nt; tf += FL) {
         const int nf = min(FL, nt - tf);
 #pragma unroll 1
@@ -644,6 +684,66 @@
   return tab ? DQ_TABLE : DQ_ARITH;
 }
 
+namespace {
+struct U8c2Plan {
+  int32_t x_limit, lut_bound, lut_rows, tchunk;
+  bool lut, lutc, one, half;
+  size_t ldsb;
+};
+U8c2Plan u8c2_plan(int in_type, int32_t T, const snnqp_conv_geom_t *g, const snnqp_weight_t *w, int nf,
+                   bool has_state, bool pl, int x_max) {
+  U8c2Plan p;
+  const bool ev1 = in_type == SNNQP_EV1;
+  const int64_t xm = (in_type == SNNQP_BITS || ev1) ? 1 : (x_max > 0 ? x_max : 1);
+  p.x_limit = (int32_t)(xm > 255 ? 255 : xm);
+  const int64_t bound = (int64_t)w->abs_sum_max * xm;
+  p.lut = w->abs_sum_max > 0 && xm > 0 && xm <= LUT_XMAX && bound <= LUT_CAP;
+  p.lut_bound = p.lut ? (int32_t)bound : 0;
+  p.tchunk = T >= TCHUNK ? TCHUNK : T;
+  const size_t lds_fixed = (size_t)p.tchunk * HIMG2 + 16 + (ev1 ? 2048 : 0) +
+                           (pl ? OutStage<true>::BYTES : OutStage<false>::BYTES);
+  const int64_t stack = w->ch_stack_max > 0 ? (int64_t)w->ch_stack_max : 8 * (int64_t)w->abs_sum_max;
+  const int64_t crows = stack * xm + 4;
+  p.lutc = p.lut && in_type != SNNQP_BITS && crows <= LUT2_ROWS && xm <= 7 &&
+           w->code_max > 0 && w->code_max <= 15;
+  p.lut_rows = p.lutc ? (int32_t)crows : 0;
+  p.one = false;
+  p.half = false;
+  p.ldsb = 0;
+  if (in_type == SNNQP_BITS) return p;
+  const int lm = p.lutc ? LUT_CHANNEL : p.lut ? LUT_SHARED : LUT_NONE;
+  const size_t lds_rest = lds_fixed - (size_t)p.tchunk * HIMG2 + u8c2_table_bytes(lm, p.lut_bound, p.lut_rows);
+  for (int wgs = 4; wgs >= 2; --wgs) {
+    const size_t per_wg = (size_t)(160 * 1024) / wgs - 512;
+    int tc = p.tchunk;
+    while (tc > 16 && (size_t)tc * HIMG2 + lds_rest > per_wg) tc -= 1;
+    if ((size_t)tc * HIMG2 + lds_rest <= per_wg) {
+      p.tchunk = tc;
+      break;
+    }
+  }
+  p.ldsb = (size_t)p.tchunk * HIMG2 + lds_rest;
+  p.one = !has_state && T <= p.tchunk;
+  p.half = event_half_group_enabled() && ev1 && p.one && p.lutc && nf == NF_MUL0 && w->cout_fire > 0 &&
+           w->cout_fire % 16 == 0 && w->cout_fire + 16 == g->Cout && g->Cout % 32 == 0;
+  return p;
+}
+}
+
+int conv3x3_event_half_group(int in_type, int32_t T, const snnqp_conv_geom_t *g, const snnqp_weight_t *w,
+                             const snnqp_neuron_t *nrn, bool has_state, int pool, int x_max) {
+  SNNQP_REQUIRE(g && w && nrn, SNNQP_EINVAL, "conv_event_half_group: null descriptor");
+  SNNQP_REQUIRE(pool == 1 || pool == 2, SNNQP_EINVAL, "conv_event_half_group: pool must be 1 or 2");
+  SNNQP_REQUIRE(T >= 0, SNNQP_EINVAL, "conv_event_half_group: negative T");
+  if (in_type != SNNQP_EV1 || T == 0) return 0;
+  if (conv3x3_mfma_unsupported(in_type, g, w, nullptr, nrn, SNNQP_BITS)) return 0;
+  SNNQP_REQUIRE(w->L >= 1.0f, SNNQP_EINVAL, "dequant L must be >= 1");
+  SNNQP_REQUIRE(w->cout_fire == 0 || (w->cout_fire > 0 && w->cout_fire % 16 == 0 && w->cout_fire <= g->Cout),
+                SNNQP_EINVAL, "conv_event_half_group: cout_fire %d is not a multiple of 16 in (0, Cout = %d]",
+                w->cout_fire, g->Cout);
+  return u8c2_plan(in_type, T, g, w, neuron_form(make_neuron(nrn)), has_state, pool == 2, x_max).half ? 1 : 0;
+}
+
 int run_conv3x3_mfma(const void *x, int in_type, int64_t xs_t, int64_t xs_b,
                      int32_t T, int32_t B, const snnqp_conv_geom_t *g,
                      const snnqp_weight_t *w, const int8_t *wt,
@@ -661,6 +761,9 @@
   SNNQP_REQUIRE(T >= 0 && B >= 0, SNNQP_EINVAL, "conv3x3 mfma: negative T/B");
   SNNQP_REQUIRE(w->L >= 1.0f, SNNQP_EINVAL, "dequant L must be >= 1");
   SNNQP_CHECK_BN(bn);
+  SNNQP_REQUIRE(w->cout_fire == 0 || (w->cout_fire > 0 && w->cout_fire % 16 == 0 && w->cout_fire <= g->Cout),
+                SNNQP_EINVAL, "conv3x3 mfma: cout_fire %d is not a multiple of 16 in (0, Cout = %d]",
+                w->cout_fire, g->Cout);
   if (T == 0 || B == 0) return SNNQP_OK;
   SNNQP_REQUIRE((int64_t)B * ((g->H + 3) / 4) * ((g->W + 7) / 8) < ((int64_t)1 << 30),
                 SNNQP_EUNSUPPORTED, "conv3x3 mfma: more than 2^30 patches in one launch");
@@ -676,6 +779,7 @@
   a.x_seen = x_seen;
   a.x_flags = nullptr;
   a.pred = pred;
+  a.cout_fire = w->cout_fire > 0 ? w->cout_fire : g->Cout;
   if (in_type == SNNQP_F32) {
     SNNQP_REQUIRE(x_flags != nullptr && (((uintptr_t)x) & 7) == 0 && xs_t % 2 == 0 && xs_b % 2 == 0,
                   SNNQP_EINVAL, "conv3x3 mfma: float32 frames need x_flags and 8-byte aligned pixels");
@@ -689,19 +793,12 @@
   const bool pl = pool == 2;
   const unsigned gy = (unsigned)((g->Cout + 127) / 128);
   const bool ev1 = in_type == SNNQP_EV1;
-  const int64_t xm = (in_type == SNNQP_BITS || ev1) ? 1 : (x_max > 0 ? x_max : 1);
-  a.x_limit = (int32_t)(xm > 255 ? 255 : xm);
-  const int64_t bound = (int64_t)w->abs_sum_max * xm;
-  const bool lut = w->abs_sum_max > 0 && xm > 0 && xm <= LUT_XMAX && bound <= LUT_CAP;
-  a.lut_bound = lut ? (int32_t)bound : 0;
-  a.tchunk = T >= TCHUNK ? TCHUNK : T;
-  const size_t lds_fixed = (size_t)a.tchunk * HIMG2 + 16 + (ev1 ? 2048 : 0) +
-                           (pl ? OutStage<true>::BYTES : OutStage<false>::BYTES);
-  const int64_t stack = w->ch_stack_max > 0 ? (int64_t)w->ch_stack_max : 8 * (int64_t)w->abs_sum_max;
-  const int64_t crows = stack * xm + 4;
-  const bool lutc = lut && in_type != SNNQP_BITS && crows <= LUT2_ROWS && xm <= 7 &&
-                    w->code_max > 0 && w->code_max <= 15;
-  a.lut_rows = lutc ? (int32_t)crows : 0;
+  const U8c2Plan plan = u8c2_plan(in_type, T, g, w, nf, u0 || u_out, pl, x_max);
+  const bool lut = plan.lut, lutc = plan.lutc;
+  a.x_limit = plan.x_limit;
+  a.lut_bound = plan.lut_bound;
+  a.tchunk = plan.tchunk;
+  a.lut_rows = plan.lut_rows;
   a.ch_slots = lutc && w->ch_stack_max > 0 ? w->ch_slots : nullptr;
 #define SNNQP_CONV_LAUNCH_IN(KERN, NFV, PL, LM, LDS)                               \
   do {                                                                             \
@@ -742,22 +839,15 @@
     const int cin_walk = conv_k16_enabled() && cin16 + 16 == cin_pad ? cin16 : cin_pad;
     launch_conv3x3_bits(a, cin_walk, i8, nf, pl, dq, fma, bnf, gy, st);
   } else {
-    const int lm = lutc ? LUT_CHANNEL : lut ? LUT_SHARED : LUT_NONE;
     if (lut) check_code_bound_once(stream_device(st), (const int8_t *)w->w, (int64_t)9 * g->Cin, g->Cout,
                                    w->abs_sum_max, st);
-    const size_t lds_rest = lds_fixed - (size_t)a.tchunk * HIMG2 + u8c2_table_bytes(lm, a.lut_bound, a.lut_rows);
-    for (int wgs = 4; wgs >= 2; --wgs) {
-      const size_t per_wg = (size_t)(160 * 1024) / wgs - 512;
-      int tc = a.tchunk;
-      while (tc > 16 && (size_t)tc * HIMG2 + lds_rest > per_wg) tc -= 1;
-      if ((size_t)tc * HIMG2 + lds_rest <= per_wg) {
-        a.tchunk = tc;
-        break;
-      }
-    }
-    const size_t ldsb = (size_t)a.tchunk * HIMG2 + lds_rest;
-    const bool one = !a.u0 && !a.u_out && a.T <= a.tchunk;
-    if (lutc) SNNQP_CONV_LAUNCH(conv3x3_u8c2_kernel, LUT_CHANNEL, ldsb);
+    const size_t ldsb = plan.ldsb;
+    const bool one = plan.one;
+    if (plan.half && pl)
+      launch_persistent(conv3x3_u8c2_kernel<NF_MUL0, true, LUT_CHANNEL, SNNQP_EV1, true, true>, a, gy, st, ldsb);
+    else if (plan.half)
+      launch_persistent(conv3x3_u8c2_kernel<NF_MUL0, false, LUT_CHANNEL, SNNQP_EV1, true, true>, a, gy, st, ldsb);
+    else if (lutc) SNNQP_CONV_LAUNCH(conv3x3_u8c2_kernel, LUT_CHANNEL, ldsb);
     else if (lut) SNNQP_CONV_LAUNCH(conv3x3_u8c2_kernel, LUT_SHARED, ldsb);
     else SNNQP_CONV_LAUNCH(conv3x3_u8c2_kernel, LUT_NONE, ldsb);
   }
diff --git a/snnquantprune_amd/csrc/conv_tile.h b/snnquantprune_amd/csrc/conv_tile.h
--- a/snnquantprune_amd/csrc/conv_tile.h
+++ b/snnquantprune_amd/csrc/conv_tile.h
@@ -81,6 +81,7 @@
   uint32_t *status;
   int32_t patch_h;
   const int32_t *pred;
+  int32_t cout_fire;
 };
 
 constexpr int SCHED_Y = 8;
@@ -183,6 +184,7 @@
   for (int k = 0; k < (slot & 3); ++k) st += (int)scr[(slot & ~3) + k];
   return st;
 }
+template <bool TWIN = false>
 __device__ __forceinline__ uint32_t build_lut_channel(float *lut, const uint32_t *scr, int max_rows,
                                                       const Dequant &dq, const BnP &bn, int cout0,
                                                       int Cout, int tid) {
@@ -192,7 +194,8 @@
   const int st = lut_column_start(scr, slot);
   const int rows = (int)scr[slot], negx = (int)scr[128 + c];
   if (st + rows > max_rows) return minbits;
-  const int co = cout0 + c < Cout ? cout0 + c : Cout - 1;
+  int co = cout0 + c < Cout ? cout0 + c : Cout - 1;
+  if (TWIN && cout0 + c >= Cout - 16 && cout0 + c < Cout) co -= 16;
   float bm = 0.f, bmul = 1.f, bb = 0.f;
   if (bn.mean) { bm = bn.mean[co]; bmul = bn.mul[co]; bb = bn.bias[co]; }
   for (int i = hf; i < rows; i += 2) {
@@ -321,7 +324,7 @@
   return tile_neurons<NF, POOL, LUTM == LUT_CHANNEL, FMA>(y, u, lc, nrn);
 }
 
-template <int NF, bool POOL, int LUTM, bool FMA = false, bool OFFS = false>
+template <int NF, bool POOL, int LUTM, bool FMA = false, bool OFFS = false, bool HALFW = false>
 __device__ __forceinline__ uint32_t tile_epilogue_halves(const v16i &acc, float (&u)[16],
                                                          const Dequant &dq, const LaneConsts &lc,
                                                          const NeuronP &nrn, int lane, float off = 0.0f) {
@@ -336,7 +339,18 @@
       const int i = 8 * g + 2 * j;
       unsigned long long m0, m1;
       neuron_pair<NF, LUTM == LUT_CHANNEL, FMA>(y[j], u[i], u[i + 1], lc, nrn, m0, m1);
-      if (POOL) {
+      if (HALFW && POOL) {
+        const unsigned long long o = m0 | m1;
+        const uint32_t lo = (uint32_t)o, hi = (uint32_t)(o >> 32);
+        myw = writelane_u32((lo | (lo >> 16)) & 0xFFFFu, 8 * g + j, myw);
+        myw = writelane_u32((hi | (hi >> 16)) & 0xFFFFu, 8 * g + 4 + j, myw);
+      } else if (HALFW) {
+#pragma unroll
+        for (int r = 0; r < 4; ++r) {
+          myw = writelane_u32((uint32_t)(m0 >> (16 * r)) & 0xFFFFu, (4 * g + r) * 8 + 2 * j, myw);
+          myw = writelane_u32((uint32_t)(m1 >> (16 * r)) & 0xFFFFu, (4 * g + r) * 8 + 2 * j + 1, myw);
+        }
+      } else if (POOL) {
         const unsigned long long o = m0 | m1;
         const uint32_t pw = (uint32_t)o | (uint32_t)(o >> 32);
         myw = writelane_u32(pw, i >> 1, myw);
@@ -474,5 +488,6 @@
 void launch_conv3x3_bits(const ConvMfmaArgs &a, int cin_walk, bool i8, int nf, bool pool, int dq,
                          bool fma, bool bnf, unsigned gy, hipStream_t st);
 bool conv_k16_enabled();
-
-}
+bool event_half_group_enabled();
+
+}
diff --git a/snnquantprune_amd/csrc/kernels.h b/snnquantprune_amd/csrc/kernels.h
--- a/snnquantprune_amd/csrc/kernels.h
+++ b/snnquantprune_amd/csrc/kernels.h
@@ -25,6 +25,8 @@
 int run_current_min(const snnqp_weight_t *w, const snnqp_bn_t *bn, int32_t bound, int32_t Cout,
                     uint32_t *out_bits, hipStream_t st);
 int conv3x3_bits_dequant_form(const snnqp_weight_t *w, const snnqp_neuron_t *nrn);
+int conv3x3_event_half_group(int in_type, int32_t T, const snnqp_conv_geom_t *g, const snnqp_weight_t *w,
+                             const snnqp_neuron_t *nrn, bool has_state, int pool, int x_max);
 int run_conv3x3_mfma(const void *x, int in_type, int64_t xs_t, int64_t xs_b,
                      int32_t T, int32_t B, const snnqp_conv_geom_t *g,
                      const snnqp_weight_t *w, const int8_t *wt,
diff --git a/snnquantprune_amd/linen.py b/snnquantprune_amd/linen.py
--- a/snnquantprune_amd/linen.py
+++ b/snnquantprune_amd/linen.py
@@ -120,6 +120,16 @@
 def conv_k16() -> bool:
   from . import _lib
   return bool(_lib.lib().snnqp_set_conv_k16(-1))
+
+
+def set_event_half_group(enabled: bool):
+  from . import _lib
+  _lib.lib().snnqp_set_event_half_group(1 if enabled else 0)
+
+
+def event_half_group() -> bool:
+  from . import _lib
+  return bool(_lib.lib().snnqp_set_event_half_group(-1))
 
 
 _TRAIN_CONV_MFMA = True
diff --git a/snnquantprune_amd/ops.py b/snnquantprune_amd/ops.py
--- a/snnquantprune_amd/ops.py
+++ b/snnquantprune_amd/ops.py
@@ -318,6 +318,7 @@
   ch_stack_max: int = 0
   ch_slots: Optional[torch.Tensor] = None
   wt_cin: int = 0
+  cout_fire: int = 0
 
   def struct(self) -> L.WeightT:
     st = self.__dict__.get("_cstruct")
@@ -327,7 +328,8 @@
                      None if self.col_sum is None else self.col_sum.data_ptr(),
                      None if self.wt6 is None else self.wt6.data_ptr(),
                      int(self.min_current_bits), int(self.ch_stack_max),
-                     None if self.ch_slots is None else self.ch_slots.data_ptr(), int(self.wt_cin))
+                     None if self.ch_slots is None else self.ch_slots.data_ptr(), int(self.wt_cin),
+                     int(self.cout_fire))
       self.__dict__["_cstruct"] = st
     return st
 
@@ -894,6 +896,10 @@
   if _PROFILE is not None and logical is not None:
     PROFILE_NOTES.setdefault(tag, {})["channels"] = {
         "cin": geom.Cin, "cout": geom.Cout, "live_out": int(logical[2])}
+    if weight.cout_fire and packed_out:
+      ev1 = L.EV1 if (in_type == L.EV1 or (binary_first and in_type in (L.U8, L.F32))) else in_type
+      PROFILE_NOTES[tag]["channels"]["half_group"] = conv_event_half_group(
+          ev1, T, geom, weight, neuron, state=u0 is not None or want_u, pool=pool, x_max=1 if ev1 == L.EV1 else x_max)
   speculate = (binary_first and packed_out and not isinstance(x, (PackedFrames, PackedSpikes))
                and in_type in (L.U8, L.F32) and geom.Cin == 2 and weight.is_int and impl != L.IMPL_GENERIC
                and xt.ndim == 5)
@@ -1086,6 +1092,16 @@
 DQ_FORMS = {1: "arith", 2: "one", 3: "table"}
 
 
+def conv_event_half_group(in_type: int, T: int, geom: ConvGeom, w: Weight, nrn: Neuron, state: bool = False,
+                          pool: int = 1, x_max: int = 0) -> bool:
+  gs, ws, ns = geom.struct(), w.struct(), nrn.struct()
+  rc = L.lib().snnqp_conv_event_half_group(int(in_type), int(T), ctypes.byref(gs), ctypes.byref(ws),
+                                           ctypes.byref(ns), 1 if state else 0, int(pool), int(x_max))
+  if rc < 0:
+    L.check(rc)
+  return rc == 1
+
+
 def conv_dequant_form(w: Weight, nrn: Neuron) -> str:
   ws, ns = w.struct(), nrn.struct()
   rc = L.lib().snnqp_conv_dequant_form(ctypes.byref(ws), ctypes.byref(ns))
diff --git a/snnquantprune_amd/packing.py b/snnquantprune_amd/packing.py
--- a/snnquantprune_amd/packing.py
+++ b/snnquantprune_amd/packing.py
@@ -57,17 +57,29 @@
   return slots, worst
 
 
-def _int_weight_of(codes: torch.Tensor, Lq: float, m: float) -> ops.Weight:
+def half_group_ranges(ranges, cout_fire: int):
+  import numpy as np
+  r = np.array(ranges, np.int64)
+  cf = int(cout_fire)
+  if cf >= 16 and cf + 16 == r.size:
+    r[cf:] = np.maximum(r[cf:], r[cf - 16:cf])
+  return r
+
+
+def _int_weight_of(codes: torch.Tensor, Lq: float, m: float, cout_fire: int = 0) -> ops.Weight:
   c2 = codes.reshape(-1, codes.shape[-1]).to(torch.int32)
   side = torch.maximum(c2.clamp(min=0).sum(0).max(), (-c2).clamp(min=0).sum(0).max())
   stats = torch.stack([side, c2.abs().max()]).tolist()
   col = c2.sum(0).to(torch.int32).contiguous() if codes.ndim == 2 else None
   slots, stack = None, 0
   if codes.ndim == 4 and codes.shape[2] == 2:
-    slots, stack = table_slots(c2.abs().sum(0).cpu().numpy())
+    slots, stack = table_slots(half_group_ranges(c2.abs().sum(0).cpu().numpy(), cout_fire))
     slots = torch.from_numpy(slots).to(codes.device)
+  else:
+    cout_fire = 0
   return ops.Weight(L.W_I8, codes, Lq, m, abs_sum_max=int(stats[0]),
-                    code_max=int(stats[1]), col_sum=col, ch_stack_max=stack, ch_slots=slots)
+                    code_max=int(stats[1]), col_sum=col, ch_stack_max=stack, ch_slots=slots,
+                    cout_fire=int(cout_fire))
 
 
 def conv_cin_pad(cin: int, kpack: bool = True) -> int:
@@ -103,12 +115,12 @@
     self._int = _int_weight_of(codes, d.L, d.m)
     return self._int
 
-  def sliced(self, rows, cols) -> "PackedKernel":
+  def sliced(self, rows, cols, cout_fire: int = 0) -> "PackedKernel":
     base = self.int_weight()
     assert base is not None, "only integer codes are sliced"
     import numpy as np
     key = ("_sliced", None if rows is None else np.asarray(rows).tobytes(),
-           None if cols is None else np.asarray(cols).tobytes())
+           None if cols is None else np.asarray(cols).tobytes(), int(cout_fire))
     pk = self._wt.get(key)
     if pk is None:
       codes = base.w
@@ -117,7 +129,7 @@
         codes = codes.index_select(codes.ndim - 2, torch.as_tensor(np.asarray(rows), device=dev))
       if cols is not None:
         codes = codes.index_select(codes.ndim - 1, torch.as_tensor(np.asarray(cols), device=dev))
-      pk = self._wt[key] = _SlicedKernel(codes.contiguous(), self.desc, base)
+      pk = self._wt[key] = _SlicedKernel(codes.contiguous(), self.desc, base, cout_fire)
     return pk
 
   def host_codes(self):
@@ -190,16 +202,16 @@
         wt6 = ops.pack_codes_fp6(codes, n_pad)
       w = ops.Weight(L.W_I8, codes, base.L, base.m, wt=wt, abs_sum_max=base.abs_sum_max,
                      code_max=base.code_max, col_sum=base.col_sum, wt6=wt6, ch_stack_max=base.ch_stack_max,
-                     ch_slots=base.ch_slots, wt_cin=wt_cin)
+                     ch_slots=base.ch_slots, wt_cin=wt_cin, cout_fire=base.cout_fire)
       self._wt[key] = w
     return w
 
 
 class _SlicedKernel(PackedKernel):
 
-  def __init__(self, codes: torch.Tensor, desc, base: ops.Weight):
+  def __init__(self, codes: torch.Tensor, desc, base: ops.Weight, cout_fire: int = 0):
     super().__init__(codes, desc, None)
-    self._int = _int_weight_of(codes, base.L, base.m)
+    self._int = _int_weight_of(codes, base.L, base.m, cout_fire)
     self._int_done = True
 
   def float_weight(self):
diff --git a/snnquantprune_amd/prune_utils.py b/snnquantprune_amd/prune_utils.py
--- a/snnquantprune_amd/prune_utils.py
+++ b/snnquantprune_amd/prune_utils.py
@@ -172,6 +172,11 @@
   return np.concatenate([idx, pad]).astype(np.int64)
 
 
+def half_group_fire(n_live: int, n_computed: int) -> int:
+  fire = -(-int(n_live) // 16) * 16
+  return fire if 0 < fire < int(n_computed) else 0
+
+
 def _host_codes(leaf, bits):
   f = np.float32
   w = _np(leaf["kernel"]).astype(f)
diff --git a/snnquantprune_amd/spiking_learning.py b/snnquantprune_amd/spiking_learning.py
--- a/snnquantprune_amd/spiking_learning.py
+++ b/snnquantprune_amd/spiking_learning.py
@@ -337,7 +337,11 @@
                                     self.norm_fn.coeffs(conn.features) if self.norm_fn is not None else None,
                                     x_bound, cmap_in)
     if rows is not None or cmap_out is not None:
-      pk = pk.sliced(rows, None if cmap_out is None else cmap_out.index)
+      fire = 0
+      if cmap_out is not None and cin == 2:
+        from . import prune_utils
+        fire = prune_utils.half_group_fire(int(cmap_out.live.sum()), int(cmap_out.index.size))
+      pk = pk.sliced(rows, None if cmap_out is None else cmap_out.index, fire)
     w = None
     if integer:
       if is_dense:
```

Result: faster. 98890 samples/s (median of 6 runs) (+2.9%).
